# yjtang249/MIPSFusion

Hardware: NVIDIA B200
Metric: map_step_rays_per_s (higher is better)
Workload: dtype f32 (decoder contractions as bf16x3 hi/lo splits on tcgen05, fp32 accumulate; encodings, render, losses, Adam in fp32)

## Files before the change

mipsfusion_b200/csrc/field_kernels.cu:

```cuda
#include "field_bwd.cuh"
#include "field_launch.cuh"
#include "field_tc_launch.cuh"
#include "field_tc_bwd.cuh"
#include "field_tc_bwd2.cuh"
#include "field_tc_bwd3.cuh"

__device__ __forceinline__ void mlp_prepare_simt(const float* __restrict__ mlp, float* __restrict__ prep, int i) {
    if (i >= PREP_SIMT_SIZE) return;
    float v = 0.f;
    if (i < MF_MLP_PARAMS) {
        v = mlp[i];
    } else if (i >= PREP_F1) {
        int r;
        if (i < PREP_B1) {
            int off, K, Kreal;
            if (i < PREP_F2) { r = i - PREP_F1; off = OFF_W1; K = D_E; Kreal = D_E; }
            else if (i < PREP_F3) { r = i - PREP_F2; off = OFF_W2; K = D_H; Kreal = D_H; }
            else { r = i - PREP_F3; off = OFF_WS1; K = D_SDF_IN; Kreal = D_SDF_IN; }
            const int k = r >> 7, tx = (r >> 3) & 15, i8 = r & 7;
            const int n = tx + 16 * i8;
            v = (k < Kreal) ? mlp[off + n * K + k] : 0.f;
        } else {
            int off, K, KI;
            if (i < PREP_B2) { r = i - PREP_B1; off = OFF_W1; K = D_E; KI = 4; }
            else if (i < PREP_B3) { r = i - PREP_B2; off = OFF_W2; K = D_H; KI = 8; }
            else { r = i - PREP_B3; off = OFF_WS1; K = D_SDF_IN; KI = 6; }
            const int n = r / (16 * KI), rem = r % (16 * KI), tx = rem / KI, ii = rem % KI;
            const int k = tx + 16 * ii;
            v = (k < K) ? mlp[off + n * K + k] : 0.f;
        }
    }
    prep[i] = v;
}

__device__ __forceinline__ void mlp_prepare_tc(const float* __restrict__ mlp, uint8_t* __restrict__ img, int t) {
    if (t < 128 * 320) {
        const int n = t / 320, kk = t % 320;
        float w; int hi_off, lo_off, k;
        if (kk < 64) {
            k = kk; const int e = tc_e_slot_to_index(k);
            w = e >= 0 ? mlp[OFF_W1 + n * D_E + e] : 0.f;
            hi_off = IMG_W1_HI; lo_off = IMG_W1_LO;
        } else if (kk < 192) {
            k = kk - 64; w = mlp[OFF_W2 + n * D_H + k];
            hi_off = IMG_W2_HI; lo_off = IMG_W2_LO;
        } else {
            k = kk - 192; w = k < D_SDF_IN ? mlp[OFF_WS1 + n * D_SDF_IN + k] : 0.f;
            hi_off = IMG_W3_HI; lo_off = IMG_W3_LO;
        }
        const __nv_bfloat16 h = __float2bfloat16_rn(w);
        const __nv_bfloat16 l = __float2bfloat16_rn(w - __bfloat162float(h));
        const uint32_t off = (uint32_t)(k >> 6) * IMG_BLOCK + sw128_offset(n, k & 63);
        *reinterpret_cast<__nv_bfloat16*>(img + hi_off + off) = h;
        *reinterpret_cast<__nv_bfloat16*>(img + lo_off + off) = l;
    } else if (t < 128 * 320 + F_COUNT) {
        const int j = t - 128 * 320;
        float v = 0.f;
        if (j < F_B2) v = mlp[OFF_B1 + j];
        else if (j < F_BS1) v = mlp[OFF_B2 + (j - F_B2)];
        else if (j < F_WR_EMB) v = mlp[OFF_BS1 + (j - F_BS1)];
        else if (j < F_WR_E) { const int c = (j - F_WR_EMB) / 64, k = (j - F_WR_EMB) % 64; v = mlp[OFF_WR + c * D_RGB_IN + k]; }
        else if (j < F_BR) {
            const int c = (j - F_WR_E) / 64, e = tc_e_slot_to_index((j - F_WR_E) % 64);
            v = e >= 0 ? mlp[OFF_WR + c * D_RGB_IN + 64 + e] : 0.f;
        }
        else if (j < F_WS2) v = (j - F_BR) < 3 ? mlp[OFF_BR + (j - F_BR)] : 0.f;
        else if (j < F_BS2) v = mlp[OFF_WS2 + (j - F_WS2)];
        else v = (j - F_BS2) < 5 ? mlp[OFF_BS2 + (j - F_BS2)] : 0.f;
        reinterpret_cast<float*>(img + IMG_F32)[j] = v;
    }
}

constexpr int PREP_BLOCKS_SIMT = (PREP_SIMT_SIZE + 255) / 256;
constexpr int PREP_BLOCKS_TC = (128 * 320 + F_COUNT + 255) / 256;
__global__ void __launch_bounds__(256) mlp_prepare_kernel(const float* __restrict__ mlp, float* __restrict__ prep) {
    if (blockIdx.x < PREP_BLOCKS_SIMT) mlp_prepare_simt(mlp, prep, blockIdx.x * 256 + threadIdx.x);
    else mlp_prepare_tc(mlp, reinterpret_cast<uint8_t*>(prep + PREP_TC), (blockIdx.x - PREP_BLOCKS_SIMT) * 256 + threadIdx.x);
}

__global__ void __launch_bounds__(NT, 2) mlp_fwd_kernel(const float* embed, const float* embed_pos, const float* pts,
                                                        const float* __restrict__ prep, float* __restrict__ out, int64_t N) {
    extern __shared__ __align__(16) float sm[];
    const int64_t n_tiles = (N + TP - 1) / TP;
    for (int64_t tile = blockIdx.x; tile < n_tiles; tile += gridDim.x) {
        load_features_tile(embed, embed_pos, pts, tile, N, sm);
        __syncthreads();
        mlp_forward_tile<false>(prep, sm, sm + ROW_H1 * LDA);
        __syncthreads();
        store_raw_tile(sm + ROW_OUT * LDA, LDA, TP, out, tile, N, threadIdx.x, NT);
        __syncthreads();
    }
}

template <class Src, bool WANT_DX>
__global__ void __launch_bounds__(NT, 1) field_bwd_kernel(FieldDev f, Src src, const float* __restrict__ d_raw,
                                                          float* __restrict__ grad_grid, float* __restrict__ part,
                                                          float* __restrict__ d_pts, int64_t N_all, ActiveMap am) {
    extern __shared__ __align__(16) float sm[];
    float* gpart = part + (size_t)blockIdx.x * MF_MLP_PARAMS;
    for (int i = threadIdx.x; i < MF_MLP_PARAMS; i += NT) gpart[i] = 0.f;
    __syncthreads();
    const int64_t N = am.n(N_all);
    const int64_t n_tiles = (N + TP - 1) / TP;
    for (int64_t tile = blockIdx.x; tile < n_tiles; tile += gridDim.x) {
        encode_tile(f, src, tile, N, sm, am);
        __syncthreads();
        mlp_forward_tile<false>(f.prep, sm, sm + ROW_H3 * LDA);
        __syncthreads();
        head_backward_tile(d_raw, tile, N, sm, am);
        __syncthreads();
        mlp_backward_tile<WANT_DX>(f.prep, sm, gpart);
        encode_backward_tile<Src, WANT_DX>(f, src, tile, N, sm, grad_grid, d_pts, am);
        __syncthreads();
    }
}

template <class Src>
__global__ void __launch_bounds__(NT, 1) field_bwd_dx_kernel(FieldDev f, Src src, const float* __restrict__ d_raw,
                                                             float* __restrict__ d_pts, int64_t N_all, ActiveMap am) {
    extern __shared__ __align__(16) float sm[];
    const int64_t N = am.n(N_all);
    const int64_t n_tiles = (N + TP - 1) / TP;
    for (int64_t tile = blockIdx.x; tile < n_tiles; tile += gridDim.x) {
        encode_tile(f, src, tile, N, sm, am);
        __syncthreads();
        mlp_forward_tile<false>(f.prep, sm, sm + ROW_H3 * LDA);
        __syncthreads();
        head_backward_tile(d_raw, tile, N, sm, am);
        __syncthreads();
        mlp_backward_tile<true, false>(f.prep, sm, nullptr);
        encode_backward_tile<Src, true, false>(f, src, tile, N, sm, nullptr, d_pts, am);
        __syncthreads();
    }
}

template <bool WANT_DX>
__global__ void __launch_bounds__(NT, 1) mlp_bwd_kernel(const float* embed, const float* embed_pos, const float* pts,
                                                        const float* __restrict__ prep, const float* __restrict__ d_out,
                                                        float* __restrict__ part, float* __restrict__ d_embed,
                                                        float* __restrict__ d_embed_pos, float* __restrict__ d_pts, int64_t N) {
    extern __shared__ __align__(16) float sm[];
    float* gpart = part + (size_t)blockIdx.x * MF_MLP_PARAMS;
    for (int i = threadIdx.x; i < MF_MLP_PARAMS; i += NT) gpart[i] = 0.f;
    __syncthreads();
    const int64_t n_tiles = (N + TP - 1) / TP;
    for (int64_t tile = blockIdx.x; tile < n_tiles; tile += gridDim.x) {
        load_features_tile(embed, embed_pos, pts, tile, N, sm);
        __syncthreads();
        mlp_forward_tile<false>(prep, sm, sm + ROW_H3 * LDA);
        __syncthreads();
        head_backward_tile(d_out, tile, N, sm);
        __syncthreads();
        mlp_backward_tile<WANT_DX>(prep, sm, gpart);
        const float* E = sm + ROW_E * LDA; const float* G = sm + ROW_G * LDA;
        const int64_t base = tile * TP;
        const int nv = (int)min((int64_t)TP, N - base);
        if (d_embed)
            for (int idx = threadIdx.x; idx < nv * D_GRID; idx += NT)
                d_embed[base * D_GRID + idx] = G[(idx % D_GRID) * LDA + idx / D_GRID];
        if (WANT_DX) {
            if (d_embed_pos)
                for (int idx = threadIdx.x; idx < nv * D_FREQ; idx += NT)
                    d_embed_pos[base * D_FREQ + idx] = E[(3 + idx % D_FREQ) * LDA + idx / D_FREQ];
            if (d_pts)
                for (int idx = threadIdx.x; idx < nv * 3; idx += NT) d_pts[base * 3 + idx] = E[(idx % 3) * LDA + idx / 3];
        }
        __syncthreads();
    }
}

__global__ void __launch_bounds__(256) reduce_partials_kernel(const float* __restrict__ part, int n_cta, float* __restrict__ grad_mlp,
                                                              int transposed, const float* __restrict__ mlp) {
    __shared__ float acc[8][32];
    if (transposed == 2 && blockIdx.x == gridDim.x - 1) {
        __shared__ float dbs1[D_H], dbr[4];
        const int t = threadIdx.x;
        if (t < D_H + 3) {
            const int sidx = t < D_H ? OFF_BS1 + t : OFF_BR + (t - D_H);
            float s = 0.f;
            for (int c = 0; c < n_cta; ++c) s += __ldg(&part[(size_t)c * MF_MLP_PARAMS + sidx]);
            if (t < D_H) dbs1[t] = s; else dbr[t - D_H] = s;
        }
        __syncthreads();
        if (t < D_H) {
            float s = 0.f;
            if (t < D_SDF_EMB) {
                for (int m = 0; m < D_H; ++m) s = fmaf(dbs1[m], __ldg(&mlp[OFF_WS1 + m * D_SDF_IN + t]), s);
            } else {
                for (int c = 0; c < 3; ++c) s = fmaf(dbr[c], __ldg(&mlp[OFF_WR + c * D_RGB_IN + (t - D_SDF_EMB)]), s);
            }
            grad_mlp[OFF_B2 + t] += s;
        }
        return;
    }
    const int lane = threadIdx.x & 31, j = threadIdx.x >> 5;
    const int sidx = blockIdx.x * 32 + lane;
    const bool on = sidx < MF_MLP_PARAMS;
    float s = 0.f;
    if (on) {
#pragma unroll 4
        for (int c = j; c < n_cta; c += 8) s += __ldg(&part[(size_t)c * MF_MLP_PARAMS + sidx]);
    }
    acc[j][lane] = s;
    __syncthreads();
    const bool b2_entry = transposed == 2 && sidx >= OFF_B2 && sidx < OFF_B2 + D_H;
    if (j == 0 && on && !b2_entry) {
        const float tot = ((acc[0][lane] + acc[1][lane]) + (acc[2][lane] + acc[3][lane])) + ((acc[4][lane] + acc[5][lane]) + (acc[6][lane] + acc[7][lane]));
        int dst = sidx;
        if (transposed) {
            if (sidx < OFF_B1) { const int r = sidx - OFF_W1; dst = OFF_W1 + (r % D_H) * D_E + r / D_H; }
            else if (sidx >= OFF_W2 && sidx < OFF_B2) { const int r = sidx - OFF_W2; dst = OFF_W2 + (r % D_H) * D_H + r / D_H; }
            else if (sidx >= OFF_WS1 && sidx < OFF_BS1) { const int r = sidx - OFF_WS1; dst = OFF_WS1 + (r % D_H) * D_SDF_IN + r / D_H; }
        }
        grad_mlp[dst] += tot;
    }
}

__global__ void ray_grad_reduce_kernel(const float* __restrict__ d_pts, const float* __restrict__ z,
                                       float* __restrict__ d_o, float* __restrict__ d_d, int64_t R, int S) {
    const int64_t r = (int64_t)blockIdx.x * (blockDim.x >> 5) + (threadIdx.x >> 5);
    const int lane = threadIdx.x & 31;
    if (r >= R) return;
    float so[3] = {0.f, 0.f, 0.f}, sd[3] = {0.f, 0.f, 0.f};
    for (int s = lane; s < S; s += 32) {
        const float zz = z[r * S + s];
#pragma unroll
        for (int k = 0; k < 3; ++k) {
            const float g = d_pts[(r * S + s) * 3 + k];
            so[k] += g; sd[k] = fmaf(zz, g, sd[k]);
        }
    }
#pragma unroll
    for (int k = 0; k < 3; ++k) { so[k] = warp_sum(so[k]); sd[k] = warp_sum(sd[k]); }
    if (lane == 0) {
#pragma unroll
        for (int k = 0; k < 3; ++k) { d_o[r * 3 + k] = so[k]; d_d[r * 3 + k] = sd[k]; }
    }
}

__global__ void hashgrid_fwd_kernel(FieldDev f, const float* __restrict__ x, float* __restrict__ out,
                                    uint32_t* __restrict__ idx_dump, int64_t N) {
    const int64_t t = (int64_t)blockIdx.x * blockDim.x + threadIdx.x;
    const int L = f.n_levels;
    if (t >= N * L) return;
    const int64_t i = t / L; const int l = (int)(t % L);
    const float xv[3] = {x[i * 3], x[i * 3 + 1], x[i * 3 + 2]};
    uint32_t idx[8];
    const float2 v = grid_level_fwd(xv, reinterpret_cast<const float2*>(f.grid), level_info(f, l), idx);
    reinterpret_cast<float2*>(out)[t] = v;
    if (idx_dump) {
#pragma unroll
        for (int c = 0; c < 8; ++c) idx_dump[t * 8 + c] = idx[c];
    }
}

template <bool WANT_DX>
__global__ void hashgrid_bwd_kernel(FieldDev f, const float* __restrict__ x, const float* __restrict__ dy,
                                    float* __restrict__ grad, float* __restrict__ dx_out, int64_t N) {
    const int64_t t = (int64_t)blockIdx.x * blockDim.x + threadIdx.x;
    const int L = f.n_levels;
    const bool active = t < N * L;
    const int64_t i = active ? t / L : 0; const int l = (int)(t % L);
    float dx[3] = {0.f, 0.f, 0.f};
    if (active) {
        const float xv[3] = {x[i * 3], x[i * 3 + 1], x[i * 3 + 2]};
        const float2 g = reinterpret_cast<const float2*>(dy)[t];
        grid_level_bwd<WANT_DX>(xv, g, reinterpret_cast<const float2*>(f.grid), grad, level_info(f, l), dx);
    }
    if (WANT_DX) {
#pragma unroll
        for (int d = 0; d < 3; ++d)
#pragma unroll
            for (int o = 8; o > 0; o >>= 1) dx[d] += __shfl_xor_sync(0xffffffffu, dx[d], o);
        if (active && l == 0) { dx_out[i * 3] = dx[0]; dx_out[i * 3 + 1] = dx[1]; dx_out[i * 3 + 2] = dx[2]; }
    }
}

__global__ void freq_fwd_kernel(const float* __restrict__ x, float* __restrict__ out, int D, int K, int64_t N) {
    const int64_t t = (int64_t)blockIdx.x * blockDim.x + threadIdx.x;
    const int W = D * K * 2;
    if (t >= N * W) return;
    const int64_t i = t / W; const int j = (int)(t % W);
    const int d = j / (2 * K), k = (j / 2) % K, s = j & 1;
    out[t] = sinf(freq_arg(x[i * D + d], k, s));
}

__global__ void freq_bwd_kernel(const float* __restrict__ x, const float* __restrict__ dy, float* __restrict__ dx,
                                int D, int K, int64_t N) {
    const int64_t t = (int64_t)blockIdx.x * blockDim.x + threadIdx.x;
    if (t >= N * D) return;
    const int64_t i = t / D; const int d = (int)(t % D);
    const float xv = x[t];
    float s = 0.f;
    for (int k = 0; k < K; ++k)
        for (int ph = 0; ph < 2; ++ph)
            s += dy[i * (D * K * 2) + d * 2 * K + 2 * k + ph] * cosf(freq_arg(xv, k, ph)) * ldexpf(3.14159274101257324f, k);
    dx[t] = s;
}

int mf_field_to_dev(const mf_field* f, FieldDev* d) {
    if (!f || !f->grid || !f->mlp_prep) { mf_set_error("mf_field: null grid/mlp_prep"); return MF_ERR_INVALID; }
    if (f->meta.n_levels != 16 || f->meta.n_features != 2) {
        mf_set_error("fused field kernels are built for 16 levels x 2 features (got %d x %d)", f->meta.n_levels, f->meta.n_features);
        return MF_ERR_UNSUPPORTED;
    }
    d->grid = f->grid; d->prep = f->mlp_prep; d->feat = nullptr;
    d->tc_img = reinterpret_cast<const uint8_t*>(f->mlp_prep + PREP_TC);
    for (int k = 0; k < 3; ++k) { d->na[k] = f->norm_a[k]; d->nb[k] = f->norm_b[k]; }
    d->nf = f->norm_factor;
    for (int l = 0; l < f->meta.n_levels; ++l)
        if (f->meta.offset[l] & 1u) { mf_set_error("mf_field: level offsets must be even (16-byte reductions)"); return MF_ERR_INVALID; }
    d->impl = f->decoder_impl == 0 ? mf_decoder_impl() : (f->decoder_impl == 1 ? 1 : 0);
    d->n_levels = f->meta.n_levels;
    for (int l = 0; l < MF_MAX_LEVELS; ++l) {
        d->scale[l] = f->meta.scale[l]; d->res[l] = f->meta.resolution[l]; d->size[l] = f->meta.size[l];
        d->offset[l] = f->meta.offset[l]; d->hashed[l] = f->meta.hashed[l];
    }
    return MF_OK;
}

static int meta_to_dev(const mf_grid_meta* m, const float* grid, FieldDev* d) {
    if (!m || m->n_levels < 1 || m->n_levels > MF_MAX_LEVELS || m->n_features != 2) {
        mf_set_error("hash grid: need 1..16 levels and 2 features per level");
        return MF_ERR_UNSUPPORTED;
    }
    memset(d, 0, sizeof(*d));
    d->grid = grid; d->n_levels = m->n_levels; d->nf = 1.0;
    for (int l = 0; l < m->n_levels; ++l) {
        d->scale[l] = m->scale[l]; d->res[l] = m->resolution[l]; d->size[l] = m->size[l];
        d->offset[l] = m->offset[l]; d->hashed[l] = m->hashed[l];
    }
    return MF_OK;
}

MF_API int mf_hashgrid_meta(int log2_T, int n_levels, int n_features, int base_res, double per_level_scale, mf_grid_meta* m) {
    MF_CHECK_ARG(m != nullptr);
    MF_CHECK_ARG(n_levels >= 1 && n_levels <= MF_MAX_LEVELS);
    MF_CHECK_ARG(log2_T >= 1 && log2_T <= 30);
    memset(m, 0, sizeof(*m));
    m->n_levels = n_levels; m->n_features = n_features; m->log2_hashmap_size = log2_T; m->base_resolution = base_res;
    const float log2_pls = log2f((float)per_level_scale);
    uint32_t off = 0;
    for (int l = 0; l < n_levels; ++l) {
        const float arg = (float)l * log2_pls;
        const float s = (float)exp2((double)arg) * (float)base_res - 1.0f;
        const uint32_t r = (uint32_t)ceilf(s) + 1u;
        const uint32_t max_params = UINT32_MAX / 2;
        uint32_t n = (powf((float)r, 3.0f) > (float)max_params) ? max_params : r * r * r;
        n = (n + 7u) / 8u * 8u;
        const uint32_t cap = 1u << log2_T;
        if (n > cap) n = cap;
        uint32_t stride = 1;
        for (int d = 0; d < 3 && stride <= n; ++d) stride *= r;
        m->scale[l] = s; m->resolution[l] = r; m->size[l] = n; m->offset[l] = off; m->hashed[l] = (n < stride) ? 1u : 0u;
        off += n;
    }
    m->offset[n_levels] = off;
    return MF_OK;
}

MF_API int mf_hashgrid_fwd(const float* x, const float* grid, const mf_grid_meta* meta, float* out, uint32_t* idx_dump,
                           int64_t N, void* stream) {
    MF_CHECK_ARG(N >= 0);
    if (N == 0) return MF_OK;
    MF_CHECK_ARG(x && grid && out);
    FieldDev d; int rc = meta_to_dev(meta, grid, &d); if (rc) return rc;
    const int64_t T = N * d.n_levels;
    hashgrid_fwd_kernel<<<(unsigned)((T + 255) / 256), 256, 0, (cudaStream_t)stream>>>(d, x, out, idx_dump, N);
    MF_LAUNCH_CHECK();
    return MF_OK;
}

MF_API int mf_hashgrid_bwd(const float* x, const float* dL_dy, const float* grid, const mf_grid_meta* meta,
                           float* grad_grid, float* dL_dx, int64_t N, void* stream) {
    MF_CHECK_ARG(N >= 0);
    if (N == 0) return MF_OK;
    MF_CHECK_ARG(x && dL_dy && grid && grad_grid);
    MF_CHECK_ARG(((uintptr_t)grad_grid & 15) == 0);
    FieldDev d; int rc = meta_to_dev(meta, grid, &d); if (rc) return rc;
    for (int l = 0; l < d.n_levels; ++l) MF_CHECK_ARG((d.offset[l] & 1u) == 0);
    if (dL_dx && d.n_levels != 16) { mf_set_error("mf_hashgrid_bwd: input gradient needs 16 levels"); return MF_ERR_UNSUPPORTED; }
    const int64_t T = N * d.n_levels;
    const unsigned blocks = (unsigned)((T + 255) / 256);
    if (dL_dx) hashgrid_bwd_kernel<true><<<blocks, 256, 0, (cudaStream_t)stream>>>(d, x, dL_dy, grad_grid, dL_dx, N);
    else hashgrid_bwd_kernel<false><<<blocks, 256, 0, (cudaStream_t)stream>>>(d, x, dL_dy, grad_grid, nullptr, N);
    MF_LAUNCH_CHECK();
    return MF_OK;
}

MF_API int mf_freq_fwd(const float* x, float* out, int n_dims, int n_frequencies, int64_t N, void* stream) {
    MF_CHECK_ARG(N >= 0 && n_dims > 0 && n_frequencies > 0);
    if (N == 0) return MF_OK;
    MF_CHECK_ARG(x && out);
    const int64_t T = N * n_dims * n_frequencies * 2;
    freq_fwd_kernel<<<(unsigned)((T + 255) / 256), 256, 0, (cudaStream_t)stream>>>(x, out, n_dims, n_frequencies, N);
    MF_LAUNCH_CHECK();
    return MF_OK;
}

MF_API int mf_freq_bwd(const float* x, const float* dL_dy, float* dL_dx, int n_dims, int n_frequencies, int64_t N, void* stream) {
    MF_CHECK_ARG(N >= 0 && n_dims > 0 && n_frequencies > 0);
    if (N == 0) return MF_OK;
    MF_CHECK_ARG(x && dL_dy && dL_dx);
    const int64_t T = N * n_dims;
    freq_bwd_kernel<<<(unsigned)((T + 255) / 256), 256, 0, (cudaStream_t)stream>>>(x, dL_dy, dL_dx, n_dims, n_frequencies, N);
    MF_LAUNCH_CHECK();
    return MF_OK;
}

MF_API int64_t mf_mlp_prep_size(void) { return PREP_SIZE; }

MF_API int mf_mlp_prepare(const float* mlp, float* mlp_prep, void* stream) {
    MF_CHECK_ARG(mlp && mlp_prep);
    mlp_prepare_kernel<<<PREP_BLOCKS_SIMT + PREP_BLOCKS_TC, 256, 0, (cudaStream_t)stream>>>(mlp, mlp_prep);
    MF_LAUNCH_CHECK();
    return MF_OK;
}

MF_API int64_t mf_mlp_grad_workspace_size(void) { return (int64_t)mf_sm_count_cached() * MF_MLP_PARAMS; }

MF_API int mf_mlp_fwd(const float* embed, const float* embed_pos, const float* pts, const float* mlp_prep, float* out,
                      int64_t N, void* stream) {
    MF_CHECK_ARG(N >= 0);
    if (N == 0) return MF_OK;
    MF_CHECK_ARG(embed && embed_pos && pts && mlp_prep && out);
    int rc = set_smem(mlp_fwd_kernel, SMEM_FWD); if (rc) return rc;
    mlp_fwd_kernel<<<persistent_grid(N, 2), NT, SMEM_FWD, (cudaStream_t)stream>>>(embed, embed_pos, pts, mlp_prep, out, N);
    MF_LAUNCH_CHECK();
    return MF_OK;
}

MF_API int mf_mlp_bwd(const float* embed, const float* embed_pos, const float* pts, const float* mlp_prep,
                      const float* d_out, float* grad_mlp, float* d_embed, float* d_embed_pos, float* d_pts,
                      float* workspace, int64_t N, void* stream) {
    MF_CHECK_ARG(N >= 0);
    if (N == 0) return MF_OK;
    MF_CHECK_ARG(embed && embed_pos && pts && mlp_prep && d_out && grad_mlp && workspace);
    const bool want_dx = d_embed_pos || d_pts;
    const int grid = persistent_grid(N, 1);
    cudaStream_t st = (cudaStream_t)stream;
    if (want_dx) {
        int rc = set_smem(mlp_bwd_kernel<true>, SMEM_BWD); if (rc) return rc;
        mlp_bwd_kernel<true><<<grid, NT, SMEM_BWD, st>>>(embed, embed_pos, pts, mlp_prep, d_out, workspace, d_embed, d_embed_pos, d_pts, N);
    } else {
        int rc = set_smem(mlp_bwd_kernel<false>, SMEM_BWD); if (rc) return rc;
        mlp_bwd_kernel<false><<<grid, NT, SMEM_BWD, st>>>(embed, embed_pos, pts, mlp_prep, d_out, workspace, d_embed, nullptr, nullptr, N);
    }
    MF_LAUNCH_CHECK();
    reduce_partials_kernel<<<(MF_MLP_PARAMS + 31) / 32, 256, 0, st>>>(workspace, grid, grad_mlp, 0, nullptr);
    MF_LAUNCH_CHECK();
    return MF_OK;
}

constexpr int ACT_BLK = 1024;

__global__ void __launch_bounds__(ACT_BLK) active_count_kernel(const float* __restrict__ d_raw, int64_t N,
                                                               uint32_t* __restrict__ flags, int* __restrict__ blk_cnt) {
    const int64_t i = (int64_t)blockIdx.x * ACT_BLK + threadIdx.x;
    bool on = false;
    if (i < N) {
        const float2* g = reinterpret_cast<const float2*>(d_raw + i * MF_RAW_DIM);
#pragma unroll
        for (int k = 0; k < MF_RAW_DIM / 2; ++k) { const float2 v = __ldg(g + k); on |= (v.x != 0.f) | (v.y != 0.f); }
    }
    const uint32_t word = __ballot_sync(0xffffffffu, on);
    if ((threadIdx.x & 31) == 0) flags[i >> 5] = word;
    const int total = __syncthreads_count(on);
    if (threadIdx.x == 0) blk_cnt[blockIdx.x] = total;
}

__global__ void __launch_bounds__(ACT_BLK) active_fill_kernel(const uint32_t* __restrict__ flags, const int* __restrict__ blk_cnt,
                                                              int* __restrict__ idx, int* __restrict__ n_active) {
    __shared__ int wsum[32];
    __shared__ int base_s;
    const int tid = threadIdx.x, lane = tid & 31, warp = tid >> 5;
    int part = 0;
    for (int j = tid; j < (int)blockIdx.x; j += ACT_BLK) part += blk_cnt[j];
#pragma unroll
    for (int o = 16; o > 0; o >>= 1) part += __shfl_xor_sync(0xffffffffu, part, o);
    if (lane == 0) wsum[warp] = part;
    __syncthreads();
    if (warp == 0) {
        int v = wsum[lane];
#pragma unroll
        for (int o = 16; o > 0; o >>= 1) v += __shfl_xor_sync(0xffffffffu, v, o);
        if (lane == 0) base_s = v;
    }
    __syncthreads();
    const int base = base_s;
    const int64_t i = (int64_t)blockIdx.x * ACT_BLK + tid;
    const uint32_t word = flags[i >> 5];
    __syncthreads();
    if (lane == 0) wsum[warp] = __popc(word);
    __syncthreads();
    if (warp == 0) {
        const int c = wsum[lane];
        int v = c;
#pragma unroll
        for (int o = 1; o < 32; o <<= 1) { const int t = __shfl_up_sync(0xffffffffu, v, o); if (lane >= o) v += t; }
        wsum[lane] = v - c;
        if (lane == 31 && blockIdx.x == gridDim.x - 1) *n_active = base + v;
    }
    __syncthreads();
    if ((word >> lane) & 1u) idx[base + wsum[warp] + __popc(word & ((1u << lane) - 1u))] = (int)i;
}

static inline int64_t act_blocks(int64_t N) { return (N + ACT_BLK - 1) / ACT_BLK; }
static inline int64_t act_scratch_words(int64_t N) { return N + act_blocks(N) * 33 + 4; }

static int compact_active_points(const float* d_raw, int64_t N, float* scratch, ActiveMap* am, cudaStream_t st) {
    if ((uintptr_t)d_raw & 7) { mf_set_error("backward: the upstream gradient must be 8-byte aligned"); return MF_ERR_INVALID; }
    if (N >= (int64_t)1 << 31) { mf_set_error("backward: more than 2^31 points"); return MF_ERR_INVALID; }
    const int64_t nb = act_blocks(N);
    int* idx = reinterpret_cast<int*>(scratch);
    uint32_t* flags = reinterpret_cast<uint32_t*>(idx + N);
    int* blk_cnt = reinterpret_cast<int*>(flags + nb * 32);
    int* count = blk_cnt + nb;
    active_count_kernel<<<(unsigned)nb, ACT_BLK, 0, st>>>(d_raw, N, flags, blk_cnt);
    MF_LAUNCH_CHECK();
    active_fill_kernel<<<(unsigned)nb, ACT_BLK, 0, st>>>(flags, blk_cnt, idx, count);
    MF_LAUNCH_CHECK();
    am->idx = idx; am->count = count;
    return MF_OK;
}

static inline int64_t cta_scratch_words() { return (int64_t)mf_sm_count_cached() * b2::SCR_CTA_WORDS; }

MF_API int64_t mf_field_bwd_workspace_size(int64_t n_points, int want_point_grads) {
    if (n_points < 0) n_points = 0;
    return mf_mlp_grad_workspace_size() + (want_point_grads ? 3 * n_points : 0) + act_scratch_words(n_points) + cta_scratch_words();
}

template <class Src>
static int launch_field_bwd(const FieldDev& d, const Src& src, const float* d_raw, float* grad_grid, float* grad_mlp,
                            float* d_pts, float* workspace, float* scratch, int64_t N, cudaStream_t st) {
    ActiveMap am{nullptr, nullptr};
    int rc0 = compact_active_points(d_raw, N, scratch, &am, st); if (rc0) return rc0;
    if (d_pts) MF_CUDA(cudaMemsetAsync(d_pts, 0, (size_t)N * 3 * sizeof(float), st));
    const bool params = grad_grid != nullptr;
    if (!params && !d_pts) {
        mf_set_error("backward without parameter gradients needs a ray / point gradient output");
        return MF_ERR_INVALID;
    }
    if (!params && d.impl == 1) {
        const int grid = persistent_grid(N, 1);
        int rc = set_smem(field_bwd_dx_kernel<Src>, SMEM_BWD); if (rc) return rc;
        field_bwd_dx_kernel<Src><<<grid, NT, SMEM_BWD, st>>>(d, src, d_raw, d_pts, N, am);
        MF_LAUNCH_CHECK();
        return MF_OK;
    }
    if (d.impl != 1) {
        const int64_t tiles = (N + TC_TP - 1) / TC_TP;
        const int64_t cap = mf_sm_count_cached();
        const int grid = (int)(tiles < cap ? (tiles > 0 ? tiles : 1) : cap);
        mf_ktimer_begin(1, st);
        if (!params) {
            int rc = set_smem(field_bwd_tc_kernel<Src, true, false>, SMEM_TC_BWD); if (rc) return rc;
            field_bwd_tc_kernel<Src, true, false><<<grid, TC_NT, SMEM_TC_BWD, st>>>(d, src, d_raw, nullptr, nullptr, d_pts, N, am, mf_tc_error_flag(), mf_tc_profile_buffer());
            mf_ktimer_end(1, st);
            MF_LAUNCH_CHECK();
            return MF_OK;
        }
        if (!d_pts && mf_bwd_impl() != 1) {
            uint32_t* cta_scr = reinterpret_cast<uint32_t*>(scratch + act_scratch_words(N));
            if (mf_bwd_impl() == 3 && d.feat) {
                int rc = set_smem(field_bwd_tc3_kernel<Src>, b3::SMEM); if (rc) return rc;
                field_bwd_tc3_kernel<Src><<<grid, b3::B3_NT, b3::SMEM, st>>>(d, src, d_raw, grad_grid, workspace, cta_scr, N, am, mf_tc_error_flag(), mf_tc_profile_buffer());
            } else {
                int rc = set_smem(field_bwd_tc2_kernel<Src>, b2::SMEM); if (rc) return rc;
                field_bwd_tc2_kernel<Src><<<grid, b2::B2_NT, b2::SMEM, st>>>(d, src, d_raw, grad_grid, workspace, cta_scr, N, am, mf_tc_error_flag(), mf_tc_profile_buffer(),
                                                                             mf_bwd_impl() == 2 ? 0 : 1);
            }
            mf_ktimer_end(1, st);
            MF_LAUNCH_CHECK();
            reduce_partials_kernel<<<(MF_MLP_PARAMS + 31) / 32 + 1, 256, 0, st>>>(workspace, grid, grad_mlp, 2, d.prep);
            MF_LAUNCH_CHECK();
            return MF_OK;
        }
        if (d_pts) {
            int rc = set_smem(field_bwd_tc_kernel<Src, true>, SMEM_TC_BWD); if (rc) return rc;
            field_bwd_tc_kernel<Src, true><<<grid, TC_NT, SMEM_TC_BWD, st>>>(d, src, d_raw, grad_grid, workspace, d_pts, N, am, mf_tc_error_flag(), mf_tc_profile_buffer());
        } else {
            int rc = set_smem(field_bwd_tc_kernel<Src, false>, SMEM_TC_BWD); if (rc) return rc;
            field_bwd_tc_kernel<Src, false><<<grid, TC_NT, SMEM_TC_BWD, st>>>(d, src, d_raw, grad_grid, workspace, nullptr, N, am, mf_tc_error_flag(), mf_tc_profile_buffer());
        }
        mf_ktimer_end(1, st);
        MF_LAUNCH_CHECK();
        reduce_partials_kernel<<<(MF_MLP_PARAMS + 31) / 32, 256, 0, st>>>(workspace, grid, grad_mlp, 1, nullptr);
        MF_LAUNCH_CHECK();
        return MF_OK;
    }
    const int grid = persistent_grid(N, 1);
    if (d_pts) {
        int rc = set_smem(field_bwd_kernel<Src, true>, SMEM_BWD); if (rc) return rc;
        field_bwd_kernel<Src, true><<<grid, NT, SMEM_BWD, st>>>(d, src, d_raw, grad_grid, workspace, d_pts, N, am);
    } else {
        int rc = set_smem(field_bwd_kernel<Src, false>, SMEM_BWD); if (rc) return rc;
        field_bwd_kernel<Src, false><<<grid, NT, SMEM_BWD, st>>>(d, src, d_raw, grad_grid, workspace, nullptr, N, am);
    }
    MF_LAUNCH_CHECK();
    reduce_partials_kernel<<<(MF_MLP_PARAMS + 31) / 32, 256, 0, st>>>(workspace, grid, grad_mlp, 0, nullptr);
    MF_LAUNCH_CHECK();
    return MF_OK;
}

MF_API int mf_field_query(const float* pts, const mf_field* field, int normalize, float* out, int64_t N, void* stream) {
    MF_CHECK_ARG(N >= 0);
    if (N == 0) return MF_OK;
    MF_CHECK_ARG(pts && out);
    FieldDev d; int rc = mf_field_to_dev(field, &d); if (rc) return rc;
    SrcPoints src{pts, normalize};
    return launch_field_fwd_auto<SrcPoints, EpiRaw, false>(d, src, EpiRaw{out}, N, (cudaStream_t)stream);
}

MF_API int mf_field_query_bwd(const float* pts, const mf_field* field, int normalize, const float* d_out, float* grad_grid,
                              float* grad_mlp, float* d_pts, float* workspace, int64_t N, void* stream) {
    MF_CHECK_ARG(N >= 0);
    if (N == 0) return MF_OK;
    MF_CHECK_ARG(pts && d_out && workspace);
    MF_CHECK_ARG((grad_grid == nullptr) == (grad_mlp == nullptr));
    MF_CHECK_ARG(grad_grid || d_pts);
    MF_CHECK_ARG(((uintptr_t)grad_grid & 15) == 0);
    FieldDev d; int rc = mf_field_to_dev(field, &d); if (rc) return rc;
    SrcPoints src{pts, normalize};
    return launch_field_bwd(d, src, d_out, grad_grid, grad_mlp, d_pts, workspace, workspace + mf_mlp_grad_workspace_size(), N,
                            (cudaStream_t)stream);
}

MF_API int64_t mf_feat_cache_size(int64_t n_points) {
    return ((n_points + TC_TP - 1) / TC_TP) * (int64_t)FEAT_TILE_WORDS * 4;
}

MF_API int mf_field_query_rays(const float* rays_o, const float* rays_d, const float* z, const mf_field* field, float* raw,
                               void* feat, int64_t R, int S, void* stream) {
    MF_CHECK_ARG(R >= 0 && S > 0);
    if (R == 0) return MF_OK;
    MF_CHECK_ARG(rays_o && rays_d && z && raw);
    FieldDev d; int rc = mf_field_to_dev(field, &d); if (rc) return rc;
    d.feat = (uint32_t*)feat;
    SrcRays src{rays_o, rays_d, z, S};
    return launch_field_fwd_auto<SrcRays, EpiRaw, false>(d, src, EpiRaw{raw}, R * S, (cudaStream_t)stream, nullptr, false, 0);
}

MF_API int mf_field_query_rays_bwd(const float* rays_o, const float* rays_d, const float* z, const mf_field* field,
                                   const float* d_raw, const void* feat, float* grad_grid, float* grad_mlp, float* d_rays_o,
                                   float* d_rays_d, float* workspace, int64_t R, int S, void* stream) {
    MF_CHECK_ARG(R >= 0 && S > 0);
    if (R == 0) return MF_OK;
    MF_CHECK_ARG(rays_o && rays_d && z && d_raw && workspace);
    MF_CHECK_ARG((grad_grid == nullptr) == (grad_mlp == nullptr));
    MF_CHECK_ARG(((uintptr_t)grad_grid & 15) == 0);
    MF_CHECK_ARG((d_rays_o == nullptr) == (d_rays_d == nullptr));
    FieldDev d; int rc = mf_field_to_dev(field, &d); if (rc) return rc;
    d.feat = (uint32_t*)feat;
    SrcRays src{rays_o, rays_d, z, S};
    cudaStream_t st = (cudaStream_t)stream;
    float* d_pts = d_rays_o ? workspace + mf_mlp_grad_workspace_size() : nullptr;
    float* scratch = workspace + mf_mlp_grad_workspace_size() + (d_rays_o ? 3 * R * S : 0);
    rc = launch_field_bwd(d, src, d_raw, grad_grid, grad_mlp, d_pts, workspace, scratch, R * S, st);
    if (rc) return rc;
    if (d_rays_o) {
        ray_grad_reduce_kernel<<<(unsigned)((R + 7) / 8), 256, 0, st>>>(d_pts, z, d_rays_o, d_rays_d, R, S);
        MF_LAUNCH_CHECK();
    }
    return MF_OK;
}
```

mipsfusion_b200/csrc/field_tc.cuh:

```cuda
#pragma once
#include "grid_encode.cuh"
#include "umma.cuh"

constexpr int TC_TP = 128;
constexpr int TC_NT = 512;
constexpr int TC_LD = TC_TP + 4;
constexpr int FEAT_WORDS = 24;
constexpr int FEAT_TILE_WORDS = 4 * FEAT_WORDS * TC_TP;

constexpr int IMG_BLOCK = 16384;
constexpr int IMG_W1_HI = 0;
constexpr int IMG_W1_LO = IMG_W1_HI + IMG_BLOCK;
constexpr int IMG_W2_HI = IMG_W1_LO + IMG_BLOCK;
constexpr int IMG_W2_LO = IMG_W2_HI + 2 * IMG_BLOCK;
constexpr int IMG_W3_HI = IMG_W2_LO + 2 * IMG_BLOCK;
constexpr int IMG_W3_LO = IMG_W3_HI + 2 * IMG_BLOCK;
constexpr int IMG_F32 = IMG_W3_LO + 2 * IMG_BLOCK;
constexpr int F_B1 = 0, F_B2 = 128, F_BS1 = 256;
constexpr int F_WR_EMB = 384;
constexpr int F_WR_E = F_WR_EMB + 192;
constexpr int F_BR = F_WR_E + 192;
constexpr int F_WS2 = F_BR + 4;
constexpr int F_BS2 = F_WS2 + 640;
constexpr int F_COUNT = F_BS2 + 8;
constexpr int IMG_BYTES = IMG_F32 + F_COUNT * 4;
static_assert(IMG_BYTES % 16 == 0, "image is copied with 16-byte loads");

__host__ __device__ inline int tc_e_slot_to_index(int slot) {
    const int q = slot >> 4, jj = slot & 15;
    if (jj < 12) return 3 + 12 * q + jj;
    if (q == 0 && jj < 15) return jj - 12;
    return -1;
}

__host__ __device__ inline uint32_t sw128_offset(int row, int k) {
    return (uint32_t)((row >> 3) * 1024 + (row & 7) * 128 + ((((k >> 3) ^ (row & 7)) & 7) << 4) + (k & 7) * 2);
}

constexpr int TM_D = 0;
constexpr int TM_A_HI = 128;
constexpr int TM_A_LO = 192;
constexpr int TM_G_HI = 256;
constexpr int TM_G_LO = 272;
constexpr int TM_COLS = 512;

constexpr int TCS_IMG = 0;
constexpr int TCS_PART = ((IMG_BYTES + 127) / 128) * 128;
constexpr int TCS_OUT = TCS_PART + 40 * TC_LD * 4;
constexpr int TCS_BAR = TCS_OUT + 10 * TC_LD * 4;
constexpr int TCS_BYTES = TCS_BAR + 32;
constexpr size_t SMEM_TC = TCS_BYTES + 1024;

struct TcCtx {
    uint8_t* img; float* part; float* out; uint64_t* bar; uint32_t* tmem_ptr;
    uint32_t tmem_base, lane_base, phase;
    const float* fw;
};

__device__ __forceinline__ void tc_setup(TcCtx& c, uint8_t* smem_raw, const uint8_t* __restrict__ img_g) {
    uint8_t* base = (uint8_t*)(((uintptr_t)smem_raw + 1023) & ~(uintptr_t)1023);
    c.img = base + TCS_IMG; c.part = (float*)(base + TCS_PART); c.out = (float*)(base + TCS_OUT);
    c.bar = (uint64_t*)(base + TCS_BAR); c.tmem_ptr = (uint32_t*)(base + TCS_BAR + 8);
    c.fw = (const float*)(c.img + IMG_F32);
    const int tid = threadIdx.x;
    for (int i = tid; i < IMG_BYTES / 16; i += blockDim.x)
        reinterpret_cast<uint4*>(c.img)[i] = __ldg(reinterpret_cast<const uint4*>(img_g) + i);
    umma::fence_proxy_async();
    if ((tid >> 5) == 0) umma::tmem_alloc<TM_COLS>(c.tmem_ptr);
    if (tid == 0) { umma::mbar_init(c.bar, 1); umma::fence_barrier_init(); }
    umma::fence_before_sync();
    __syncthreads();
    umma::fence_after_sync();
    c.tmem_base = *c.tmem_ptr;
    c.lane_base = c.tmem_base + ((uint32_t)(((tid >> 5) & 3) * 32) << 16);
    c.phase = 0;
}

__device__ __forceinline__ void tc_teardown(TcCtx& c) {
    umma::fence_before_sync();
    __syncthreads();
    if ((threadIdx.x >> 5) == 0) umma::tmem_dealloc<TM_COLS>(c.tmem_base);
}

template <class ColFn>
__device__ __forceinline__ void tc_layer_mma(const TcCtx& c, int img_hi, int img_lo, int KS, ColFn a_col) {
    constexpr uint32_t idesc = umma::idesc_bf16(128, 128, 0, 0);
    const uint32_t d = c.tmem_base + TM_D;
    const uint32_t w_hi = umma::smem_u32(c.img + img_hi), w_lo = umma::smem_u32(c.img + img_lo);
    uint32_t acc = 0;
#pragma unroll 1
    for (int pass = 0; pass < 3; ++pass) {
        const bool a_is_lo = pass == 2, w_is_lo = pass == 1;
#pragma unroll 1
        for (int ks = 0; ks < KS; ++ks) {
            const uint32_t a = c.tmem_base + (uint32_t)a_col(ks, a_is_lo);
            const uint32_t wb = (w_is_lo ? w_lo : w_hi) + (uint32_t)((ks >> 2) * IMG_BLOCK + (ks & 3) * 32);
            umma::mma_ts(d, a, umma::smem_desc_sw128(wb, 16, 1024), idesc, acc);
            acc = 1;
        }
    }
}

template <class ColFn>
__device__ __forceinline__ bool tc_run_layer(TcCtx& c, int img_hi, int img_lo, int KS, ColFn a_col) {
    umma::wait_st();
    umma::fence_before_sync();
    __syncthreads();
    if (threadIdx.x == 0) {
        umma::fence_after_sync();
        tc_layer_mma(c, img_hi, img_lo, KS, a_col);
        umma::commit(c.bar);
    }
    const bool ok = umma::mbar_wait(c.bar, c.phase);
    c.phase ^= 1;
    umma::fence_after_sync();
    return ok;
}

__device__ __forceinline__ void tc_load_acc(const TcCtx& c, int q, float (&v)[32]) {
    uint32_t r[32];
    umma::tmem_ld32(c.lane_base + TM_D + 32 * q, r);
    umma::wait_ld();
#pragma unroll
    for (int i = 0; i < 32; ++i) v[i] = __uint_as_float(r[i]);
}

__device__ __forceinline__ void tc_store_act32(const TcCtx& c, int q, const float (&v)[32]) {
    uint32_t hi[16], lo[16];
#pragma unroll
    for (int i = 0; i < 16; ++i) umma::split2(v[2 * i], v[2 * i + 1], hi[i], lo[i]);
    umma::tmem_st16(c.lane_base + TM_A_HI + 16 * q, hi);
    umma::tmem_st16(c.lane_base + TM_A_LO + 16 * q, lo);
}

template <class Src, bool SDF_ONLY>
__device__ __forceinline__ void tc_encode_tile(const TcCtx& c, const FieldDev& f, const Src& src, int64_t tile, int64_t N) {
    const int tid = threadIdx.x, p = tid & (TC_TP - 1), q = tid >> 7;
    const int64_t i = tile * TC_TP + p;
    const bool valid = i < N;
    float x[3] = {0.f, 0.f, 0.f};
    if (valid) src.point(i, f, x);
    float e[16];
#pragma unroll
    for (int jj = 0; jj < 12; ++jj) {
        const int j = q * 12 + jj, d = j >> 4, k = (j & 15) >> 1, s = j & 1;
        e[jj] = sin_reduced(freq_arg(x[d], k, s));
    }
    e[12] = q == 0 ? x[0] : 0.f; e[13] = q == 0 ? x[1] : 0.f; e[14] = q == 0 ? x[2] : 0.f; e[15] = 0.f;
    {
        uint32_t hi[8], lo[8];
#pragma unroll
        for (int t = 0; t < 8; ++t) umma::split2(e[2 * t], e[2 * t + 1], hi[t], lo[t]);
        umma::tmem_st8(c.lane_base + TM_A_HI + 8 * q, hi);
        umma::tmem_st8(c.lane_base + TM_A_LO + 8 * q, lo);
        if (f.feat) {
            uint32_t* fo = f.feat + (size_t)tile * FEAT_TILE_WORDS + (size_t)q * FEAT_WORDS * TC_TP + p;
#pragma unroll
            for (int t = 0; t < 8; ++t) { fo[t * TC_TP] = hi[t]; fo[(8 + t) * TC_TP] = lo[t]; }
        }
    }
    if (!SDF_ONLY) {
        const float* wre = c.fw + F_WR_E + 16 * q;
        float r[3] = {0.f, 0.f, 0.f};
#pragma unroll
        for (int t = 0; t < 16; ++t)
#pragma unroll
            for (int ch = 0; ch < 3; ++ch) r[ch] = fmaf(wre[ch * 64 + t], e[t], r[ch]);
#pragma unroll
        for (int ch = 0; ch < 3; ++ch) c.part[(q * 3 + ch) * TC_LD + p] = r[ch];
    }
    const float2* grid2 = reinterpret_cast<const float2*>(f.grid);
    float g[8];
#pragma unroll
    for (int ll = 0; ll < 4; ++ll) {
        float2 v = make_float2(0.f, 0.f);
        if (valid) v = grid_level_fwd(x, grid2, level_info(f, q * 4 + ll), nullptr);
        g[2 * ll] = v.x; g[2 * ll + 1] = v.y;
    }
    {
        uint32_t hi[4], lo[4];
#pragma unroll
        for (int t = 0; t < 4; ++t) umma::split2(g[2 * t], g[2 * t + 1], hi[t], lo[t]);
        umma::tmem_st4(c.lane_base + TM_G_HI + 4 * q, hi);
        umma::tmem_st4(c.lane_base + TM_G_LO + 4 * q, lo);
        if (f.feat) {
            uint32_t* fo = f.feat + (size_t)tile * FEAT_TILE_WORDS + (size_t)q * FEAT_WORDS * TC_TP + p;
#pragma unroll
            for (int t = 0; t < 4; ++t) { fo[(16 + t) * TC_TP] = hi[t]; fo[(20 + t) * TC_TP] = lo[t]; }
        }
    }
}

template <bool SDF_ONLY>
__device__ __forceinline__ bool tc_mlp_forward_tile(TcCtx& c) {
    const int tid = threadIdx.x, p = tid & (TC_TP - 1), q = tid >> 7;
    bool ok = true;
    float v[32];
    ok &= tc_run_layer(c, IMG_W1_HI, IMG_W1_LO, 4, [](int ks, bool lo) { return (lo ? TM_A_LO : TM_A_HI) + 8 * ks; });
    tc_load_acc(c, q, v);
#pragma unroll
    for (int i = 0; i < 32; ++i) v[i] = fmaxf(v[i] + c.fw[F_B1 + 32 * q + i], 0.f);
    tc_store_act32(c, q, v);
    ok &= tc_run_layer(c, IMG_W2_HI, IMG_W2_LO, 8, [](int ks, bool lo) { return (lo ? TM_A_LO : TM_A_HI) + 8 * ks; });
    tc_load_acc(c, q, v);
#pragma unroll
    for (int i = 0; i < 32; ++i) v[i] += c.fw[F_B2 + 32 * q + i];
    if (q < 2) {
        tc_store_act32(c, q, v);
    } else if (!SDF_ONLY) {
        const float* wr = c.fw + F_WR_EMB + 32 * (q - 2);
        float r[3] = {0.f, 0.f, 0.f};
#pragma unroll
        for (int i = 0; i < 32; ++i)
#pragma unroll
            for (int ch = 0; ch < 3; ++ch) r[ch] = fmaf(wr[ch * 64 + i], v[i], r[ch]);
#pragma unroll
        for (int ch = 0; ch < 3; ++ch) c.part[(12 + (q - 2) * 3 + ch) * TC_LD + p] = r[ch];
    }
    ok &= tc_run_layer(c, IMG_W3_HI, IMG_W3_LO, 6, [](int ks, bool lo) {
        return ks < 4 ? (lo ? TM_A_LO : TM_A_HI) + 8 * ks : (lo ? TM_G_LO : TM_G_HI) + 8 * (ks - 4);
    });
    tc_load_acc(c, q, v);
    {
        float s[N_CLASS] = {0.f, 0.f, 0.f, 0.f, 0.f};
        const float* ws2 = c.fw + F_WS2 + 32 * q;
#pragma unroll
        for (int i = 0; i < 32; ++i) {
            const float h = fmaxf(v[i] + c.fw[F_BS1 + 32 * q + i], 0.f);
#pragma unroll
            for (int ch = 0; ch < N_CLASS; ++ch) s[ch] = fmaf(ws2[ch * 128 + i], h, s[ch]);
        }
#pragma unroll
        for (int ch = 0; ch < N_CLASS; ++ch) c.part[(18 + q * 5 + ch) * TC_LD + p] = s[ch];
    }
    umma::fence_before_sync();
    __syncthreads();
    if (q == 0) {
        const float* P = c.part;
        float zl[N_CLASS], rgb[3];
#pragma unroll
        for (int ch = 0; ch < N_CLASS; ++ch)
            zl[ch] = c.fw[F_BS2 + ch] + ((P[(18 + ch) * TC_LD + p] + P[(23 + ch) * TC_LD + p]) + (P[(28 + ch) * TC_LD + p] + P[(33 + ch) * TC_LD + p]));
#pragma unroll
        for (int ch = 0; ch < 3; ++ch)
            rgb[ch] = SDF_ONLY ? 0.f
                               : c.fw[F_BR + ch] + (((P[ch * TC_LD + p] + P[(3 + ch) * TC_LD + p]) + (P[(6 + ch) * TC_LD + p] + P[(9 + ch) * TC_LD + p])) +
                                                    (P[(12 + ch) * TC_LD + p] + P[(15 + ch) * TC_LD + p]));
        float mx = zl[0];
#pragma unroll
        for (int ch = 1; ch < N_CLASS; ++ch) mx = fmaxf(mx, zl[ch]);
        float pr[N_CLASS], se = 0.f;
#pragma unroll
        for (int ch = 0; ch < N_CLASS; ++ch) { pr[ch] = expf(zl[ch] - mx); se += pr[ch]; }
        float ent = 0.f, ex = 0.f;
#pragma unroll
        for (int ch = 0; ch < N_CLASS; ++ch) {
            pr[ch] = pr[ch] / se;
            ent += pr[ch] * log2f(pr[ch] + 1e-5f);
            ex += pr[ch] * (float)ch;
        }
        float* O = c.out;
        O[0 * TC_LD + p] = rgb[0]; O[1 * TC_LD + p] = rgb[1]; O[2 * TC_LD + p] = rgb[2];
        O[3 * TC_LD + p] = (ex / 4.0f - 0.5f) * 2.0f;
        O[4 * TC_LD + p] = -1.0f * ent;
#pragma unroll
        for (int ch = 0; ch < N_CLASS; ++ch) O[(5 + ch) * TC_LD + p] = pr[ch];
    }
    return ok;
}

template <class Src, class Epi, bool SDF_ONLY>
__global__ void __launch_bounds__(TC_NT, 1) field_fwd_tc_kernel(FieldDev f, Src src, Epi epi, int64_t N,
                                                                const unsigned int* __restrict__ n_dev,
                                                                const uint8_t* __restrict__ img, int* __restrict__ err,
                                                                long long* __restrict__ prof) {
    extern __shared__ uint8_t smem_raw[];
#define TC_MARK(k) do { if (prof && threadIdx.x == 0 && blockIdx.x == 0 && tile == (int64_t)gridDim.x) prof[32 + (k)] = clock64(); } while (0)
    if (n_dev) N = (int64_t)*n_dev;
    TcCtx c;
    tc_setup(c, smem_raw, img);
    bool ok = true;
    const int64_t n_tiles = (N + TC_TP - 1) / TC_TP;
    for (int64_t tile = blockIdx.x; tile < n_tiles; tile += gridDim.x) {
        TC_MARK(0);
        tc_encode_tile<Src, SDF_ONLY>(c, f, src, tile, N);
        TC_MARK(1);
        ok &= tc_mlp_forward_tile<SDF_ONLY>(c);
        TC_MARK(2);
        __syncthreads();
        epi.store(c.out, TC_LD, TC_TP, tile, N, threadIdx.x, TC_NT);
        __syncthreads();
        TC_MARK(3);
    }
    if (!ok && err) atomicExch(err, 1);
    tc_teardown(c);
}
```

mipsfusion_b200/csrc/field_tc3.cuh:

```cuda
#pragma once
#include "field_tc.cuh"

constexpr int T3_GT = 256;
constexpr int T3_D = 0, T3_A_HI = 128, T3_A_LO = 192, T3_STG = 256, T3_STG_COLS = 96;
constexpr int T3_E_HI = 0, T3_E_LO = 32, T3_G_HI = 64, T3_G_LO = 80;
constexpr int T3_CPART_ROWS = 6;
constexpr int T3_PART_ROWS = 13;
constexpr int T3S_CPART = ((IMG_BYTES + 127) / 128) * 128;
constexpr int T3S_PART = T3S_CPART + 2 * T3_CPART_ROWS * TC_LD * 4;
constexpr int T3S_OUT = T3S_PART + T3_PART_ROWS * TC_LD * 4;
constexpr int T3S_BAR = T3S_OUT + MF_RAW_DIM * TC_LD * 4;
constexpr size_t SMEM_TC3 = T3S_BAR + 64 + 1024;
static_assert(SMEM_TC3 <= 227 * 1024, "shared memory budget");

__device__ __forceinline__ void t3_cons_sync() { asm volatile("bar.sync 1, %0;" ::"n"(T3_GT) : "memory"); }

struct T3Cons {
    uint8_t* img; const float* fw; float* part; float* out; uint64_t* bar;
    uint32_t tmem, lane_base, phase;
    int tid;
    bool ok;
};

template <int KS, int N_OUT = 128, class ColFn, class AfterFn>
__device__ __forceinline__ void t3_run_layer(T3Cons& c, int img_hi, int img_lo, ColFn a_col, AfterFn after_issue) {
    umma::wait_st();
    umma::fence_before_sync();
    t3_cons_sync();
    if (c.tid == 0) {
        umma::fence_after_sync();
        constexpr uint32_t idesc = umma::idesc_bf16(128, N_OUT, 0, 0);
        const uint64_t dh = umma::smem_desc_sw128(umma::smem_u32(c.img + img_hi), 16, 1024);
        const uint64_t dl = umma::smem_desc_sw128(umma::smem_u32(c.img + img_lo), 16, 1024);
#pragma unroll
        for (int pass = 0; pass < 3; ++pass) {
#pragma unroll
            for (int ks = 0; ks < KS; ++ks) {
                const uint32_t off = (uint32_t)(((ks >> 2) * IMG_BLOCK + (ks & 3) * 32) >> 4);
                umma::mma_ts(c.tmem + T3_D, c.tmem + (uint32_t)a_col(ks, pass == 2), (pass == 1 ? dl : dh) + off, idesc, (pass | ks) ? 1u : 0u);
            }
        }
        umma::commit(c.bar);
        after_issue();
    }
    c.ok &= umma::mbar_wait(c.bar, c.phase);
    c.phase ^= 1;
    umma::fence_after_sync();
}

__device__ __forceinline__ void t3_load32(const T3Cons& c, int col, float (&v)[32]) {
    uint32_t r[32];
    umma::tmem_ld32(c.lane_base + (uint32_t)col, r);
    umma::wait_ld();
#pragma unroll
    for (int i = 0; i < 32; ++i) v[i] = __uint_as_float(r[i]);
}
__device__ __forceinline__ void t3_store32(const T3Cons& c, int f0, const float (&v)[32]) {
    uint32_t hi[16], lo[16];
#pragma unroll
    for (int i = 0; i < 16; ++i) umma::split2(v[2 * i], v[2 * i + 1], hi[i], lo[i]);
    umma::tmem_st16(c.lane_base + (uint32_t)(T3_A_HI + f0 / 2), hi);
    umma::tmem_st16(c.lane_base + (uint32_t)(T3_A_LO + f0 / 2), lo);
}

template <class Src, class Epi, bool SDF_ONLY>
__global__ void __launch_bounds__(2 * T3_GT, 1) field_fwd_tc3_kernel(FieldDev f, Src src, Epi epi, int64_t N,
                                                                     const unsigned int* __restrict__ n_dev,
                                                                     const uint8_t* __restrict__ img, int* __restrict__ err,
                                                                     long long* __restrict__ prof, int* __restrict__ tile_ctr = nullptr) {
    extern __shared__ uint8_t smem_raw[];
    __shared__ uint32_t tmem_ptr_s;
#define T3_MARK(slot) do { if (prof && blockIdx.x == 0 && tid == 0 && k == 2) prof[slot] = clock64(); } while (0)
    if (n_dev) N = (int64_t)*n_dev;
    if (prof && blockIdx.x == 0 && threadIdx.x == 0) prof[29] = clock64();
    if (prof && threadIdx.x == 0 && blockIdx.x < 256) prof[64 + 2 * blockIdx.x] = mf_globaltimer();
    uint8_t* base = (uint8_t*)(((uintptr_t)smem_raw + 1023) & ~(uintptr_t)1023);
    uint64_t* bars = (uint64_t*)(base + T3S_BAR);
    if ((threadIdx.x >> 5) == 0) umma::tmem_alloc<512>(&tmem_ptr_s);
    if (threadIdx.x == 0) {
        umma::mbar_init(bars + 0, 1);
        umma::mbar_init(bars + 1, T3_GT); umma::mbar_init(bars + 2, T3_GT);
        umma::mbar_init(bars + 3, 1); umma::mbar_init(bars + 4, 1);
        umma::mbar_init(bars + 7, 1);
        umma::fence_barrier_init();
        constexpr uint32_t CHUNK = 32768;
        asm volatile("mbarrier.arrive.expect_tx.shared::cta.b64 _, [%0], %1;" ::"r"(umma::smem_u32(bars + 7)), "r"((uint32_t)IMG_BYTES) : "memory");
        for (uint32_t off = 0; off < (uint32_t)IMG_BYTES; off += CHUNK) {
            const uint32_t nb = (uint32_t)IMG_BYTES - off < CHUNK ? (uint32_t)IMG_BYTES - off : CHUNK;
            asm volatile("cp.async.bulk.shared::cluster.global.mbarrier::complete_tx::bytes [%0], [%1], %2, [%3];"
                         ::"r"(umma::smem_u32(base + off)), "l"(img + off), "r"(nb), "r"(umma::smem_u32(bars + 7)) : "memory");
        }
    }
    umma::fence_before_sync();
    __syncthreads();
    umma::fence_after_sync();
    bool img_ok = umma::mbar_wait(bars + 7, 0);
    const uint32_t tmem = tmem_ptr_s;
    const bool producer = threadIdx.x < T3_GT;
    const int tid = threadIdx.x & (T3_GT - 1), p = tid & 127, h = tid >> 7;
    const uint32_t lane_base = tmem + ((uint32_t)(((tid >> 5) & 3) * 32) << 16);
    const float* fw = (const float*)(base + IMG_F32);
    const int64_t n_tiles = (N + TC_TP - 1) / TC_TP;
    bool ok = img_ok;
    volatile int* tq = reinterpret_cast<volatile int*>(base + T3S_BAR + 40);
    if (threadIdx.x < 4) tq[threadIdx.x] = 0;

    if (producer) {
        const float2* grid2 = reinterpret_cast<const float2*>(f.grid);
        for (uint32_t k = 0;; ++k) {
            const int s = (int)(k & 1u);
            const uint32_t stg = lane_base + (uint32_t)(T3_STG + T3_STG_COLS * s);
            float* cpart = (float*)(base + T3S_CPART) + s * T3_CPART_ROWS * TC_LD;
            T3_MARK(40);
            if (prof && blockIdx.x == 0 && tid == 0 && k < 12) prof[16 + k] = clock64();
            const int64_t tile_e = k < 2 ? (int64_t)blockIdx.x + (int64_t)k * gridDim.x : (int64_t)tq[k & 3u];
            float x[3] = {0.f, 0.f, 0.f};
            if (tile_e >= 0 && tile_e < n_tiles && tile_e * TC_TP + p < N) src.point(tile_e * TC_TP + p, f, x);
            ok &= umma::mbar_wait(bars + 3 + s, ((k >> 1) & 1u) ^ 1u);
            umma::fence_after_sync();
            const int64_t tile = k < 2 ? tile_e : (int64_t)tq[k & 3u];
            if (tile >= n_tiles) break;
            if (tid == 0) {
                const int64_t t2 = tile_ctr ? 2 * (int64_t)gridDim.x + atomicAdd(tile_ctr, 1) : tile + 2 * (int64_t)gridDim.x;
                tq[(k + 2u) & 3u] = (int)(t2 < n_tiles ? t2 : n_tiles);
            }
            const int64_t i = tile * TC_TP + p;
            const bool valid = i < N;
            if (tile != tile_e) {
                x[0] = x[1] = x[2] = 0.f;
                if (valid) src.point(i, f, x);
            }
            T3_MARK(41);
            float r[3] = {0.f, 0.f, 0.f};
#pragma unroll
            for (int sg = 0; sg < 2; ++sg) {
                const int qq = 2 * h + sg;
                float e[16];
#pragma unroll
                for (int jj = 0; jj < 12; ++jj) {
                    const int j = qq * 12 + jj, d = j >> 4, kk = (j & 15) >> 1, ph = j & 1;
                    e[jj] = sin_reduced(freq_arg(x[d], kk, ph));
                }
                e[12] = qq == 0 ? x[0] : 0.f; e[13] = qq == 0 ? x[1] : 0.f; e[14] = qq == 0 ? x[2] : 0.f; e[15] = 0.f;
                uint32_t hi[8], lo[8];
#pragma unroll
                for (int t = 0; t < 8; ++t) umma::split2(e[2 * t], e[2 * t + 1], hi[t], lo[t]);
                umma::tmem_st8(stg + T3_E_HI + 8 * qq, hi);
                umma::tmem_st8(stg + T3_E_LO + 8 * qq, lo);
                if (f.feat) {
                    uint32_t* fo = f.feat + (size_t)tile * FEAT_TILE_WORDS + (size_t)qq * FEAT_WORDS * TC_TP + p;
#pragma unroll
                    for (int t = 0; t < 8; ++t) { fo[t * TC_TP] = hi[t]; fo[(8 + t) * TC_TP] = lo[t]; }
                }
                if (!SDF_ONLY) {
                    const float* wre = fw + F_WR_E + 16 * qq;
#pragma unroll
                    for (int t = 0; t < 16; ++t)
#pragma unroll
                        for (int ch = 0; ch < 3; ++ch) r[ch] = fmaf(wre[ch * 64 + t], e[t], r[ch]);
                }
            }
            if (!SDF_ONLY) {
#pragma unroll
                for (int ch = 0; ch < 3; ++ch) cpart[(h * 3 + ch) * TC_LD + p] = r[ch];
            }
            T3_MARK(42);
#pragma unroll 1
            for (int sg = 0; sg < 2; ++sg) {
                float gf[8];
#pragma unroll 2
                for (int ll = 0; ll < 4; ++ll) {
                    float2 v2 = make_float2(0.f, 0.f);
                    if (valid) v2 = grid_level_fwd(x, grid2, level_info(f, 8 * h + 4 * sg + ll), nullptr);
                    gf[2 * ll] = v2.x; gf[2 * ll + 1] = v2.y;
                }
                uint32_t ghi[4], glo[4];
#pragma unroll
                for (int t = 0; t < 4; ++t) umma::split2(gf[2 * t], gf[2 * t + 1], ghi[t], glo[t]);
                umma::tmem_st4(stg + T3_G_HI + 8 * h + 4 * sg, ghi);
                umma::tmem_st4(stg + T3_G_LO + 8 * h + 4 * sg, glo);
                if (f.feat) {
                    uint32_t* fo = f.feat + (size_t)tile * FEAT_TILE_WORDS + (size_t)(2 * h + sg) * FEAT_WORDS * TC_TP + p;
#pragma unroll
                    for (int t = 0; t < 4; ++t) { fo[(16 + t) * TC_TP] = ghi[t]; fo[(20 + t) * TC_TP] = glo[t]; }
                }
            }
            T3_MARK(43);
            umma::wait_st();
            umma::fence_before_sync();
            umma::mbar_arrive(bars + 1 + s);
            T3_MARK(44);
        }
    } else {
        T3Cons c;
        c.img = base; c.fw = fw; c.part = (float*)(base + T3S_PART); c.out = (float*)(base + T3S_OUT); c.bar = bars;
        c.tmem = tmem; c.lane_base = lane_base; c.phase = 0; c.tid = tid; c.ok = ok;
        float v[32];
        for (uint32_t k = 0;; ++k) {
            const int64_t tile = k < 2 ? (int64_t)blockIdx.x + (int64_t)k * gridDim.x : (int64_t)tq[k & 3u];
            if (tile >= n_tiles) break;
            const int s = (int)(k & 1u);
            const int stg = T3_STG + T3_STG_COLS * s;
            const float* cpart = (const float*)(base + T3S_CPART) + s * T3_CPART_ROWS * TC_LD;
            T3_MARK(48);
            c.ok &= umma::mbar_wait(bars + 1 + s, (k >> 1) & 1u);
            umma::fence_after_sync();
            T3_MARK(49);
            float rgb_e[3] = {0.f, 0.f, 0.f};
            if (!SDF_ONLY && h == 0) {
#pragma unroll
                for (int ch = 0; ch < 3; ++ch) rgb_e[ch] = cpart[ch * TC_LD + p] + cpart[(3 + ch) * TC_LD + p];
            }
            t3_run_layer<4>(c, IMG_W1_HI, IMG_W1_LO, [stg](int ks, bool lo) { return stg + (lo ? T3_E_LO : T3_E_HI) + 8 * ks; }, []() {});
            T3_MARK(50);
#pragma unroll 1
            for (int half = 0; half < 2; ++half) {
                const int f0 = 64 * h + 32 * half;
                t3_load32(c, T3_D + f0, v);
                const float4* b4 = reinterpret_cast<const float4*>(c.fw + F_B1 + f0);
#pragma unroll
                for (int k4 = 0; k4 < 8; ++k4) {
                    const float4 b = b4[k4];
                    v[4 * k4] = fmaxf(v[4 * k4] + b.x, 0.f); v[4 * k4 + 1] = fmaxf(v[4 * k4 + 1] + b.y, 0.f);
                    v[4 * k4 + 2] = fmaxf(v[4 * k4 + 2] + b.z, 0.f); v[4 * k4 + 3] = fmaxf(v[4 * k4 + 3] + b.w, 0.f);
                }
                t3_store32(c, f0, v);
            }
            T3_MARK(51);
            if (SDF_ONLY) {
                t3_run_layer<8, 64>(c, IMG_W2_HI, IMG_W2_LO, [](int ks, bool lo) { return (lo ? T3_A_LO : T3_A_HI) + 8 * ks; }, []() {});
                T3_MARK(52);
                const int f0 = 32 * h;
                t3_load32(c, T3_D + f0, v);
                const float4* b4 = reinterpret_cast<const float4*>(c.fw + F_B2 + f0);
#pragma unroll
                for (int k4 = 0; k4 < 8; ++k4) {
                    const float4 b = b4[k4];
                    v[4 * k4] += b.x; v[4 * k4 + 1] += b.y; v[4 * k4 + 2] += b.z; v[4 * k4 + 3] += b.w;
                }
                t3_store32(c, f0, v);
            } else {
            t3_run_layer<8>(c, IMG_W2_HI, IMG_W2_LO, [](int ks, bool lo) { return (lo ? T3_A_LO : T3_A_HI) + 8 * ks; }, []() {});
            T3_MARK(52);
            {
                float r[3] = {0.f, 0.f, 0.f};
#pragma unroll 1
                for (int half = 0; half < 2; ++half) {
                    const int f0 = 64 * h + 32 * half;
                    t3_load32(c, T3_D + f0, v);
                    const float4* b4 = reinterpret_cast<const float4*>(c.fw + F_B2 + f0);
#pragma unroll
                    for (int k4 = 0; k4 < 8; ++k4) {
                        const float4 b = b4[k4];
                        v[4 * k4] += b.x; v[4 * k4 + 1] += b.y; v[4 * k4 + 2] += b.z; v[4 * k4 + 3] += b.w;
                    }
                    if (h == 0) {
                        t3_store32(c, f0, v);
                    } else {
#pragma unroll
                        for (int ch = 0; ch < 3; ++ch) {
                            const float4* w4 = reinterpret_cast<const float4*>(c.fw + F_WR_EMB + ch * 64 + 32 * half);
#pragma unroll
                            for (int k4 = 0; k4 < 8; ++k4) {
                                const float4 w = w4[k4];
                                r[ch] = fmaf(w.x, v[4 * k4], r[ch]); r[ch] = fmaf(w.y, v[4 * k4 + 1], r[ch]);
                                r[ch] = fmaf(w.z, v[4 * k4 + 2], r[ch]); r[ch] = fmaf(w.w, v[4 * k4 + 3], r[ch]);
                            }
                        }
                    }
                }
                if (h == 1) {
#pragma unroll
                    for (int ch = 0; ch < 3; ++ch) c.part[ch * TC_LD + p] = r[ch];
                }
            }
            }
            T3_MARK(53);
            uint64_t* empty = bars + 3 + s;
            t3_run_layer<6>(c, IMG_W3_HI, IMG_W3_LO,
                         [stg](int ks, bool lo) { return ks < 4 ? (lo ? T3_A_LO : T3_A_HI) + 8 * ks : stg + (lo ? T3_G_LO : T3_G_HI) + 8 * (ks - 4); },
                         [empty]() { umma::commit(empty); });
            T3_MARK(54);
            {
                float sl[N_CLASS] = {0.f, 0.f, 0.f, 0.f, 0.f};
#pragma unroll 1
                for (int half = 0; half < 2; ++half) {
                    const int f0 = 64 * h + 32 * half;
                    t3_load32(c, T3_D + f0, v);
                    const float4* b4 = reinterpret_cast<const float4*>(c.fw + F_BS1 + f0);
#pragma unroll
                    for (int k4 = 0; k4 < 8; ++k4) {
                        const float4 b = b4[k4];
                        v[4 * k4] = fmaxf(v[4 * k4] + b.x, 0.f); v[4 * k4 + 1] = fmaxf(v[4 * k4 + 1] + b.y, 0.f);
                        v[4 * k4 + 2] = fmaxf(v[4 * k4 + 2] + b.z, 0.f); v[4 * k4 + 3] = fmaxf(v[4 * k4 + 3] + b.w, 0.f);
                    }
#pragma unroll
                    for (int ch = 0; ch < N_CLASS; ++ch) {
                        const float4* w4 = reinterpret_cast<const float4*>(c.fw + F_WS2 + ch * 128 + f0);
#pragma unroll
                        for (int k4 = 0; k4 < 8; ++k4) {
                            const float4 w = w4[k4];
                            sl[ch] = fmaf(w.x, v[4 * k4], sl[ch]); sl[ch] = fmaf(w.y, v[4 * k4 + 1], sl[ch]);
                            sl[ch] = fmaf(w.z, v[4 * k4 + 2], sl[ch]); sl[ch] = fmaf(w.w, v[4 * k4 + 3], sl[ch]);
                        }
                    }
                }
#pragma unroll
                for (int ch = 0; ch < N_CLASS; ++ch) c.part[(3 + h * 5 + ch) * TC_LD + p] = sl[ch];
            }
            T3_MARK(55);
            umma::fence_before_sync();
            t3_cons_sync();
            if (h == 0) {
                const float* P = c.part;
                float zl[N_CLASS], rgb[3];
#pragma unroll
                for (int ch = 0; ch < N_CLASS; ++ch) zl[ch] = c.fw[F_BS2 + ch] + (P[(3 + ch) * TC_LD + p] + P[(8 + ch) * TC_LD + p]);
#pragma unroll
                for (int ch = 0; ch < 3; ++ch) rgb[ch] = SDF_ONLY ? 0.f : c.fw[F_BR + ch] + (rgb_e[ch] + P[ch * TC_LD + p]);
                float mx = zl[0];
#pragma unroll
                for (int ch = 1; ch < N_CLASS; ++ch) mx = fmaxf(mx, zl[ch]);
                float pr[N_CLASS], se = 0.f;
#pragma unroll
                for (int ch = 0; ch < N_CLASS; ++ch) { pr[ch] = expf(zl[ch] - mx); se += pr[ch]; }
                float ent = 0.f, ex = 0.f;
#pragma unroll
                for (int ch = 0; ch < N_CLASS; ++ch) {
                    pr[ch] = pr[ch] / se;
                    ent += pr[ch] * log2f(pr[ch] + 1e-5f);
                    ex += pr[ch] * (float)ch;
                }
                float* O = c.out;
                O[0 * TC_LD + p] = rgb[0]; O[1 * TC_LD + p] = rgb[1]; O[2 * TC_LD + p] = rgb[2];
                O[3 * TC_LD + p] = (ex / 4.0f - 0.5f) * 2.0f;
                O[4 * TC_LD + p] = -1.0f * ent;
#pragma unroll
                for (int ch = 0; ch < N_CLASS; ++ch) O[(5 + ch) * TC_LD + p] = pr[ch];
            }
            t3_cons_sync();
            T3_MARK(56);
            epi.store(c.out, TC_LD, TC_TP, tile, N, c.tid, T3_GT);
            t3_cons_sync();
            T3_MARK(57);
        }
        ok = c.ok;
    }
    if (!ok && err) atomicExch(err, 1);
    umma::fence_before_sync();
    __syncthreads();
    if (prof && blockIdx.x == 0 && threadIdx.x == 0) prof[28] = clock64();
    if (prof && threadIdx.x == 0 && blockIdx.x < 256) prof[65 + 2 * blockIdx.x] = mf_globaltimer();
    if (tile_ctr && threadIdx.x == 0 && atomicAdd(tile_ctr + 1, 1) == (int)gridDim.x - 1) {
        tile_ctr[0] = 0; tile_ctr[1] = 0;
        __threadfence();
    }
    if ((threadIdx.x >> 5) == 0) umma::tmem_dealloc<512>(tmem);
}
```

mipsfusion_b200/csrc/field_tc_bwd2.cuh:

```cuda
#pragma once
#include "field_tc_bwd.cuh"

namespace b2 {

constexpr int B2_NT = 512, CHAIN_NT = 256, WG_NT = 128, SC_NT = 128;
constexpr int QROWS = 32;
constexpr uint32_t QBLK = QROWS * 128;
constexpr int S_W = 0;
constexpr int W2H = 0, W2L = IMG_W2_LO - IMG_W2_HI, W3H = IMG_W3_HI - IMG_W2_HI, W3L = IMG_W3_LO - IMG_W2_HI;
constexpr int S_ST = IMG_F32 - IMG_W2_HI;
constexpr int ST_A = 0, ST_B = 4 * (int)QBLK, ST_BYTES = 8 * (int)QBLK;
constexpr int W1H = S_ST + IMG_W1_HI, W1L = S_ST + IMG_W1_LO;
constexpr int S_F32 = S_ST + 2 * ST_BYTES;
constexpr int S_PART = S_F32 + ((F_COUNT * 4 + 127) / 128) * 128;
constexpr int PART_ROWS = 10;
constexpr int S_BAR = S_PART + PART_ROWS * TC_LD * 4;
constexpr int S_BYTES = S_BAR + 256;
constexpr size_t SMEM = S_BYTES + 1024;
static_assert(SMEM <= 227 * 1024, "shared memory budget");
constexpr int T_D = 0, T_R1_HI = 128, T_R1_LO = 192, T_R2_HI = 256, T_R2_LO = 320, T_DW = 384;
constexpr int T_G_HI = T_R2_HI + 32, T_G_LO = T_R2_LO + 32;
constexpr int SCR_H1 = 0, SCR_H3 = 128, SCR_RGB = 256, SCR_U = 320, SCR_WORDS = 328;
constexpr int64_t SCR_CTA_WORDS = (int64_t)SCR_WORDS * TC_TP;
constexpr int REGS_CHAIN = 160, REGS_WGRAD = 88, REGS_SCATTER = 104;
enum { B_MMA = 0, B_DG3, B_DCONS, B_DWFREE, B_DWRDY, B_W1, B_IMG, B_FREE0, B_ISS0 = B_FREE0 + 4, B_COUNT = B_ISS0 + 4 };
constexpr int N_X3 = 112;

__device__ __forceinline__ void chain_sync() { asm volatile("bar.sync 1, %0;" ::"n"(CHAIN_NT) : "memory"); }
__device__ __forceinline__ void wg_sync() { asm volatile("bar.sync 2, %0;" ::"n"(WG_NT) : "memory"); }

struct Ctx {
    uint8_t* base; const float* fw; float* part; uint64_t* bars;
    uint32_t tmem, lane_base;
    bool ok;
};

template <int KS, class ColFn>
__device__ __forceinline__ void issue_fwd(const Ctx& c, int w_hi_off, int w_lo_off, ColFn a_col) {
    constexpr uint32_t idesc = umma::idesc_bf16(128, 128, 0, 0);
    const uint64_t dh = umma::smem_desc_sw128(umma::smem_u32(c.base + S_W + w_hi_off), 16, 1024);
    const uint64_t dl = umma::smem_desc_sw128(umma::smem_u32(c.base + S_W + w_lo_off), 16, 1024);
#pragma unroll
    for (int pass = 0; pass < 3; ++pass)
#pragma unroll
        for (int ks = 0; ks < KS; ++ks) {
            const uint32_t off = (uint32_t)(((ks >> 2) * IMG_BLOCK + (ks & 3) * 32) >> 4);
            umma::mma_ts(c.tmem + T_D, c.tmem + (uint32_t)a_col(ks, pass == 2), (pass == 1 ? dl : dh) + off, idesc, (pass | ks) ? 1u : 0u);
        }
}
template <int N_OUT>
__device__ __forceinline__ void issue_dgrad(const Ctx& c, int a_hi, int a_lo, int w_hi_off, int w_lo_off) {
    constexpr uint32_t idesc = umma::idesc_bf16(128, N_OUT, 0, 1);
    const uint64_t dh = umma::smem_desc_sw128(umma::smem_u32(c.base + S_W + w_hi_off), IMG_BLOCK, 1024);
    const uint64_t dl = umma::smem_desc_sw128(umma::smem_u32(c.base + S_W + w_lo_off), IMG_BLOCK, 1024);
#pragma unroll
    for (int pass = 0; pass < 3; ++pass)
#pragma unroll
        for (int ks = 0; ks < 8; ++ks)
            umma::mma_ts(c.tmem + T_D, c.tmem + (uint32_t)((pass == 2 ? a_lo : a_hi) + 8 * ks), (pass == 1 ? dl : dh) + (uint32_t)((ks * 2048) >> 4),
                         idesc, (pass | ks) ? 1u : 0u);
}

__device__ __forceinline__ void ld32f(uint32_t taddr, float (&v)[32]) {
    uint32_t r[32];
    umma::tmem_ld32(taddr, r);
    umma::wait_ld();
#pragma unroll
    for (int i = 0; i < 32; ++i) v[i] = __uint_as_float(r[i]);
}

__device__ __forceinline__ void st_op(const Ctx& c, int hi_col, int lo_col, int f0, const uint32_t (&hi)[16], const uint32_t (&lo)[16]) {
    umma::tmem_st16(c.lane_base + (uint32_t)(hi_col + f0 / 2), hi);
    umma::tmem_st16(c.lane_base + (uint32_t)(lo_col + f0 / 2), lo);
}
__device__ __forceinline__ void split32(const float (&v)[32], uint32_t (&hi)[16], uint32_t (&lo)[16]) {
#pragma unroll
    for (int i = 0; i < 16; ++i) umma::split2(v[2 * i], v[2 * i + 1], hi[i], lo[i]);
}

template <int OFF>
__device__ __forceinline__ void sts128(uint32_t addr, uint32_t a, uint32_t b, uint32_t c_, uint32_t d) {
    asm volatile("st.shared.v4.b32 [%0+%1], {%2, %3, %4, %5};" ::"r"(addr), "n"(OFF), "r"(a), "r"(b), "r"(c_), "r"(d) : "memory");
}
template <int TILE_OFF, int CC>
__device__ __forceinline__ void put32(const uint32_t (&P)[8], const uint32_t (&pk)[16]) {
#pragma unroll
    for (int c_ = 0; c_ < 4; ++c_) sts128<TILE_OFF>(P[4 * CC + c_], pk[4 * c_], pk[4 * c_ + 1], pk[4 * c_ + 2], pk[4 * c_ + 3]);
}
template <int TILE_OFF, int SG>
__device__ __forceinline__ void put16(const uint32_t (&P)[8], const uint32_t (&pk)[8]) {
#pragma unroll
    for (int c_ = 0; c_ < 2; ++c_) sts128<TILE_OFF>(P[2 * SG + c_], pk[4 * c_], pk[4 * c_ + 1], pk[4 * c_ + 2], pk[4 * c_ + 3]);
}
template <int TILE_OFF>
__device__ __forceinline__ void put64(const uint32_t (&P)[8], const uint32_t (&wh)[2][16], const uint32_t (&wl)[2][16]) {
    put32<TILE_OFF, 0>(P, wh[0]); put32<TILE_OFF, 1>(P, wh[1]);
    put32<TILE_OFF + 2 * (int)QBLK, 0>(P, wl[0]); put32<TILE_OFF + 2 * (int)QBLK, 1>(P, wl[1]);
}

__device__ __forceinline__ void scr_store(uint32_t* scr_p, int region, int lo_off, int w0, const uint32_t (&hi)[16], const uint32_t (&lo)[16]) {
#pragma unroll
    for (int t = 0; t < 16; ++t) {
        __stcg(scr_p + (size_t)(region + w0 + t) * TC_TP, hi[t]);
        __stcg(scr_p + (size_t)(region + lo_off + w0 + t) * TC_TP, lo[t]);
    }
}
__device__ __forceinline__ void scr_load(const uint32_t* scr_p, int region, int lo_off, int w0, uint32_t (&hi)[16], uint32_t (&lo)[16]) {
#pragma unroll
    for (int t = 0; t < 16; ++t) {
        hi[t] = __ldcg(scr_p + (size_t)(region + w0 + t) * TC_TP);
        lo[t] = __ldcg(scr_p + (size_t)(region + lo_off + w0 + t) * TC_TP);
    }
}

}

template <class Src>
__global__ void __launch_bounds__(b2::B2_NT, 1) field_bwd_tc2_kernel(FieldDev f, Src src, const float* __restrict__ d_raw,
                                                                  float* __restrict__ grad_grid, float* __restrict__ part,
                                                                  uint32_t* __restrict__ scratch, int64_t N_all, ActiveMap am,
                                                                  int* __restrict__ err, long long* __restrict__ prof, int agg) {
    using namespace b2;
    extern __shared__ uint8_t smem_raw[];
    const int tid = threadIdx.x, warp = tid >> 5;
    if (prof && tid == 0 && blockIdx.x < 256) prof[576 + 2 * blockIdx.x] = mf_globaltimer();
    float* gpart = part + (size_t)blockIdx.x * MF_MLP_PARAMS;
    for (int i = tid; i < MF_MLP_PARAMS; i += B2_NT) gpart[i] = 0.f;

    Ctx c;
    c.base = (uint8_t*)(((uintptr_t)smem_raw + 1023) & ~(uintptr_t)1023);
    c.fw = (const float*)(c.base + S_F32); c.part = (float*)(c.base + S_PART); c.bars = (uint64_t*)(c.base + S_BAR);
    uint32_t* tmem_ptr = (uint32_t*)(c.base + S_BAR + 8 * B_COUNT);
    if (warp == 0) umma::tmem_alloc<512>(tmem_ptr);
    if (tid == 0) {
        umma::mbar_init(c.bars + B_MMA, 1); umma::mbar_init(c.bars + B_DG3, 1); umma::mbar_init(c.bars + B_DCONS, SC_NT);
        umma::mbar_init(c.bars + B_DWFREE, WG_NT); umma::mbar_init(c.bars + B_DWRDY, 4); umma::mbar_init(c.bars + B_W1, 1);
        umma::mbar_init(c.bars + B_IMG, 1);
        for (int q = 0; q < 4; ++q) { umma::mbar_init(c.bars + B_FREE0 + q, 1); umma::mbar_init(c.bars + B_ISS0 + q, 1); }
        umma::fence_barrier_init();
        constexpr uint32_t W_BYTES = IMG_F32 - IMG_W2_HI, F_BYTES = F_COUNT * 4, CHUNK = 32768;
        asm volatile("mbarrier.arrive.expect_tx.shared::cta.b64 _, [%0], %1;" ::"r"(umma::smem_u32(c.bars + B_IMG)), "r"(W_BYTES + F_BYTES) : "memory");
        for (uint32_t off = 0; off < W_BYTES; off += CHUNK)
            asm volatile("cp.async.bulk.shared::cluster.global.mbarrier::complete_tx::bytes [%0], [%1], %2, [%3];"
                         ::"r"(umma::smem_u32(c.base + S_W + off)), "l"(f.tc_img + IMG_W2_HI + off), "r"(W_BYTES - off < CHUNK ? W_BYTES - off : CHUNK),
                           "r"(umma::smem_u32(c.bars + B_IMG)) : "memory");
        asm volatile("cp.async.bulk.shared::cluster.global.mbarrier::complete_tx::bytes [%0], [%1], %2, [%3];"
                     ::"r"(umma::smem_u32(c.base + S_F32)), "l"(f.tc_img + IMG_F32), "r"(F_BYTES), "r"(umma::smem_u32(c.bars + B_IMG)) : "memory");
    }
    umma::fence_before_sync();
    __syncthreads();
    umma::fence_after_sync();
    c.tmem = *tmem_ptr;
    c.lane_base = c.tmem + ((uint32_t)((warp & 3) * 32) << 16);
    c.ok = umma::mbar_wait(c.bars + B_IMG, 0);

    const int64_t N = am.n(N_all);
    const int64_t n_tiles = (N + TC_TP - 1) / TC_TP;
    const int p = tid & (TC_TP - 1);
#define B2_MARK(slot) do { if (prof && blockIdx.x == 0 && k == 1 && (ctid & 127) == 0) prof[slot] = clock64(); } while (0)

    const int ctid = tid - SC_NT;
    if (ctid >= 0 && ctid < CHAIN_NT) {
        asm volatile("setmaxnreg.inc.sync.aligned.u32 %0;" ::"n"(REGS_CHAIN));
        const int h = ctid >> 7;
        uint32_t ph_mma = 0;
        uint32_t k = 0;
        auto round = [&](auto issue) {
            umma::wait_st();
            umma::fence_before_sync();
            chain_sync();
            if (ctid == 0) { umma::fence_after_sync(); issue(); umma::commit(c.bars + B_MMA); }
            c.ok &= umma::mbar_wait_spin(c.bars + B_MMA, ph_mma);
            ph_mma ^= 1;
            umma::fence_after_sync();
        };
        const int row = p & (QROWS - 1), quarter = p >> 5, lane = tid & 31;
        uint32_t PA[8], PH[8], PQ[4];
#pragma unroll
        for (int j = 0; j < 8; ++j) {
            PA[j] = umma::smem_u32(c.base) + (uint32_t)(S_ST + (quarter & 1) * ST_BYTES) + (uint32_t)((row >> 3) * 1024 + (row & 7) * 128) +
                    (uint32_t)(((j ^ row) & 7) << 4);
            PH[j] = PA[j] + (uint32_t)h * QBLK;
        }
#pragma unroll
        for (int c_ = 0; c_ < 4; ++c_) PQ[c_] = h ? PA[4 + c_] : PA[c_];
        const uint64_t dA0 = umma::desc_mn(c.base + S_ST + (quarter & 1) * ST_BYTES + ST_A, 0, QBLK);
        const uint64_t dB0 = umma::desc_mn(c.base + S_ST + (quarter & 1) * ST_BYTES + ST_B, 0, QBLK);
        constexpr uint32_t LO_STEP = (2 * QBLK) >> 4, KS_STEP = (16 * 128) >> 4;
        auto prod_begin = [&](uint32_t prod) {
            c.ok &= umma::mbar_wait_spin(c.bars + B_FREE0 + ((quarter + 2) & 3), quarter >= 2 ? (prod & 1u) : ((prod + 1u) & 1u));
        };
        auto prod_end = [&](int PK, uint32_t prod, uint32_t lay) {
            umma::fence_proxy_async();
            asm volatile("bar.sync %0, 64;" ::"r"(3 + quarter) : "memory");
            if (h == 0 && lane == 0) {
                umma::fence_after_sync();
                if (quarter == 0) {
                    if (PK == 0 || PK == 2 || PK == 3) c.ok &= umma::mbar_wait_spin(c.bars + B_DWFREE, (lay + 1u) & 1u);
                } else {
                    c.ok &= umma::mbar_wait_spin(c.bars + B_ISS0 + quarter - 1, prod & 1u);
                }
                const int n_out = PK == 0 ? N_X3 : (PK == 2 ? D_H : (PK == 3 ? 64 : 16));
                const uint32_t idesc = umma::idesc_bf16(128, n_out, 1, 1);
                const uint32_t dcol = c.tmem + (uint32_t)(T_DW + (PK == 1 ? N_X3 : (PK == 4 ? 64 : 0)));
#pragma unroll
                for (int j = 0; j < 6; ++j) {
                    const int pass = j >> 1, ks = j & 1;
                    umma::mma_ss(dcol, dA0 + (uint64_t)((pass == 1 ? LO_STEP : 0) + ks * KS_STEP),
                                 dB0 + (uint64_t)((pass == 2 ? LO_STEP : 0) + ks * KS_STEP), idesc, (j == 0 && quarter == 0) ? 0u : 1u);
                }
                umma::mbar_arrive(c.bars + B_ISS0 + quarter);
                umma::commit(c.bars + B_FREE0 + quarter);
                if (PK == 1 || PK == 2 || PK == 4) umma::commit(c.bars + B_DWRDY);
            }
        };
        auto put_u = [&](const uint32_t (&uh)[4], const uint32_t (&ul)[4]) {
            if (h == 0) { sts128<ST_B>(PA[0], uh[0], uh[1], uh[2], uh[3]); sts128<ST_B>(PA[1], 0u, 0u, 0u, 0u); }
            else { sts128<ST_B + 2 * (int)QBLK>(PA[0], ul[0], ul[1], ul[2], ul[3]); sts128<ST_B + 2 * (int)QBLK>(PA[1], 0u, 0u, 0u, 0u); }
        };
        auto load_w1 = [&]() {
            umma::fence_proxy_async();
            asm volatile("mbarrier.arrive.expect_tx.shared::cta.b64 _, [%0], %1;" ::"r"(umma::smem_u32(c.bars + B_W1)), "r"(2 * IMG_BLOCK) : "memory");
            asm volatile("cp.async.bulk.shared::cluster.global.mbarrier::complete_tx::bytes [%0], [%1], %2, [%3];"
                         ::"r"(umma::smem_u32(c.base + S_ST)), "l"(f.tc_img + IMG_W1_HI), "r"(2 * IMG_BLOCK), "r"(umma::smem_u32(c.bars + B_W1))
                         : "memory");
        };
        uint32_t* scr_p = scratch + (size_t)blockIdx.x * SCR_CTA_WORDS + p;
        auto load_z = [&](int r_hi, int r_lo, uint32_t (&wh)[2][16], uint32_t (&wl)[2][16]) {
#pragma unroll
            for (int cc = 0; cc < 2; ++cc) {
                umma::tmem_ld16(c.lane_base + (uint32_t)(r_hi + 16 * (2 * h + cc)), wh[cc]);
                umma::tmem_ld16(c.lane_base + (uint32_t)(r_lo + 16 * (2 * h + cc)), wl[cc]);
            }
            umma::wait_ld();
        };

        int64_t i_next = 0;
        { const int64_t s0 = (int64_t)blockIdx.x * TC_TP + p; if (s0 < N) i_next = am(s0); }
        for (int64_t tile = blockIdx.x; tile < n_tiles; tile += gridDim.x, ++k) {
            const int64_t slot = tile * TC_TP + p;
            const bool valid = slot < N;
            const int64_t i = i_next;
            { const int64_t s1 = slot + (int64_t)gridDim.x * TC_TP; i_next = s1 < N ? am(s1) : 0; }
            const uint32_t lay0 = 3u * k, prod0 = 5u * k;
            if (ctid == 0) {
                if (k > 0) {
                    c.ok &= umma::mbar_wait_spin(c.bars + B_FREE0 + 0, (prod0 - 1u) & 1u);
                    c.ok &= umma::mbar_wait_spin(c.bars + B_FREE0 + 2, (prod0 - 1u) & 1u);
                }
                load_w1();
            }
            B2_MARK(0);
            float g[3], gs[7];
            {
                const float2* gr = reinterpret_cast<const float2*>(d_raw + i * MF_RAW_DIM);
                float2 t2[5];
#pragma unroll
                for (int j = 0; j < 5; ++j) t2[j] = valid ? __ldg(gr + j) : make_float2(0.f, 0.f);
                g[0] = t2[0].x; g[1] = t2[0].y; g[2] = t2[1].x;
                gs[0] = t2[1].y; gs[1] = t2[2].x; gs[2] = t2[2].y; gs[3] = t2[3].x; gs[4] = t2[3].y; gs[5] = t2[4].x; gs[6] = t2[4].y;
            }
            float x[3] = {0.f, 0.f, 0.f};
            if (!f.feat && valid) src.point(i, f, x);
            const uint32_t* fin = f.feat ? f.feat + (size_t)(i >> 7) * FEAT_TILE_WORDS + (i & (TC_TP - 1)) : nullptr;
            auto e_words = [&](int qq, uint32_t (&hi)[8], uint32_t (&lo)[8]) {
                if (fin) {
                    const uint32_t* fq = fin + (size_t)qq * FEAT_WORDS * TC_TP;
#pragma unroll
                    for (int t = 0; t < 8; ++t) { hi[t] = __ldg(fq + t * TC_TP); lo[t] = __ldg(fq + (8 + t) * TC_TP); }
                } else {
                    float e[16];
                    tb_e_slots(x, qq, e);
#pragma unroll
                    for (int t = 0; t < 8; ++t) umma::split2(e[2 * t], e[2 * t + 1], hi[t], lo[t]);
                }
            };
#pragma unroll
            for (int sg = 0; sg < 2; ++sg) {
                const int qq = 2 * h + sg;
                uint32_t hi[8], lo[8], gh[4], gl[4];
                e_words(qq, hi, lo);
                if (fin) {
                    const uint32_t* fq = fin + (size_t)qq * FEAT_WORDS * TC_TP;
#pragma unroll
                    for (int t = 0; t < 4; ++t) { gh[t] = __ldg(fq + (16 + t) * TC_TP); gl[t] = __ldg(fq + (20 + t) * TC_TP); }
                } else {
                    float gf[8];
                    const float2* grid2 = reinterpret_cast<const float2*>(f.grid);
#pragma unroll
                    for (int ll = 0; ll < 4; ++ll) {
                        float2 vv = make_float2(0.f, 0.f);
                        if (valid) vv = grid_level_fwd(x, grid2, level_info(f, qq * 4 + ll), nullptr);
                        gf[2 * ll] = vv.x; gf[2 * ll + 1] = vv.y;
                    }
#pragma unroll
                    for (int t = 0; t < 4; ++t) umma::split2(gf[2 * t], gf[2 * t + 1], gh[t], gl[t]);
                }
                umma::tmem_st8(c.lane_base + T_R1_HI + 8 * qq, hi);
                umma::tmem_st8(c.lane_base + T_R1_LO + 8 * qq, lo);
                umma::tmem_st4(c.lane_base + T_G_HI + 4 * qq, gh);
                umma::tmem_st4(c.lane_base + T_G_LO + 4 * qq, gl);
            }
            B2_MARK(1);
            float v[32];
            uint32_t mask1[2], mask3[2];
            round([&]() {
                c.ok &= umma::mbar_wait_spin(c.bars + B_W1, k & 1u);
                issue_fwd<4>(c, W1H, W1L, [](int ks, bool lo) { return (lo ? T_R1_LO : T_R1_HI) + 8 * ks; });
            });
#pragma unroll 1
            for (int cc = 0; cc < 2; ++cc) {
                const int f0 = 64 * h + 32 * cc;
                ld32f(c.lane_base + T_D + f0, v);
                const float4* b4 = reinterpret_cast<const float4*>(c.fw + F_B1 + f0);
                uint32_t m = 0;
#pragma unroll
                for (int k4 = 0; k4 < 8; ++k4) {
                    const float4 b = b4[k4];
                    v[4 * k4] = fmaxf(v[4 * k4] + b.x, 0.f); v[4 * k4 + 1] = fmaxf(v[4 * k4 + 1] + b.y, 0.f);
                    v[4 * k4 + 2] = fmaxf(v[4 * k4 + 2] + b.z, 0.f); v[4 * k4 + 3] = fmaxf(v[4 * k4 + 3] + b.w, 0.f);
                }
#pragma unroll
                for (int kk = 0; kk < 32; ++kk) m |= (v[kk] > 0.f ? 1u : 0u) << kk;
                mask1[cc] = m;
                uint32_t hi[16], lo[16];
                split32(v, hi, lo);
                st_op(c, T_R1_HI, T_R1_LO, f0, hi, lo);
                scr_store(scr_p, SCR_H1, 64, f0 / 2, hi, lo);
            }
            B2_MARK(2);
            round([&]() { issue_fwd<8>(c, W2H, W2L, [](int ks, bool lo) { return (lo ? T_R1_LO : T_R1_HI) + 8 * ks; }); });
#pragma unroll 1
            for (int cc = 0; cc < 2; ++cc) {
                const int f0 = 64 * h + 32 * cc;
                ld32f(c.lane_base + T_D + f0, v);
                const float4* b4 = reinterpret_cast<const float4*>(c.fw + F_B2 + f0);
#pragma unroll
                for (int k4 = 0; k4 < 8; ++k4) {
                    const float4 b = b4[k4];
                    v[4 * k4] += b.x; v[4 * k4 + 1] += b.y; v[4 * k4 + 2] += b.z; v[4 * k4 + 3] += b.w;
                }
                uint32_t hi[16], lo[16];
                split32(v, hi, lo);
                if (h == 0) st_op(c, T_R2_HI, T_R2_LO, f0, hi, lo);
                else scr_store(scr_p, SCR_RGB, 32, 16 * cc, hi, lo);
            }
            B2_MARK(3);
            round([&]() {
                issue_fwd<6>(c, W3H, W3L, [](int ks, bool lo) {
                    return ks < 4 ? (lo ? T_R2_LO : T_R2_HI) + 8 * ks : (lo ? T_G_LO : T_G_HI) + 8 * (ks - 4);
                });
            });
            {
                float s[N_CLASS] = {0.f, 0.f, 0.f, 0.f, 0.f};
#pragma unroll 1
                for (int cc = 0; cc < 2; ++cc) {
                    const int f0 = 64 * h + 32 * cc;
                    ld32f(c.lane_base + T_D + f0, v);
                    const float4* b4 = reinterpret_cast<const float4*>(c.fw + F_BS1 + f0);
                    uint32_t m = 0;
#pragma unroll
                    for (int k4 = 0; k4 < 8; ++k4) {
                        const float4 b = b4[k4];
                        v[4 * k4] = fmaxf(v[4 * k4] + b.x, 0.f); v[4 * k4 + 1] = fmaxf(v[4 * k4 + 1] + b.y, 0.f);
                        v[4 * k4 + 2] = fmaxf(v[4 * k4 + 2] + b.z, 0.f); v[4 * k4 + 3] = fmaxf(v[4 * k4 + 3] + b.w, 0.f);
                    }
#pragma unroll
                    for (int kk = 0; kk < 32; ++kk) m |= (v[kk] > 0.f ? 1u : 0u) << kk;
                    mask3[cc] = m;
#pragma unroll
                    for (int ch = 0; ch < N_CLASS; ++ch) {
                        const float4* w4 = reinterpret_cast<const float4*>(c.fw + F_WS2 + ch * 128 + f0);
#pragma unroll
                        for (int k4 = 0; k4 < 8; ++k4) {
                            const float4 w = w4[k4];
                            s[ch] = fmaf(w.x, v[4 * k4], s[ch]); s[ch] = fmaf(w.y, v[4 * k4 + 1], s[ch]);
                            s[ch] = fmaf(w.z, v[4 * k4 + 2], s[ch]); s[ch] = fmaf(w.w, v[4 * k4 + 3], s[ch]);
                        }
                    }
                    uint32_t hi[16], lo[16];
                    split32(v, hi, lo);
                    scr_store(scr_p, SCR_H3, 64, f0 / 2, hi, lo);
                }
#pragma unroll
                for (int ch = 0; ch < N_CLASS; ++ch) c.part[(h * 5 + ch) * TC_LD + p] = s[ch];
            }
            B2_MARK(4);
            chain_sync();
            float dz4[N_CLASS];
            {
                float zl[N_CLASS], pr[N_CLASS], dp[N_CLASS];
                float mx = -INFINITY, se = 0.f, dot = 0.f;
#pragma unroll
                for (int ch = 0; ch < N_CLASS; ++ch) {
                    zl[ch] = c.fw[F_BS2 + ch] + (c.part[ch * TC_LD + p] + c.part[(5 + ch) * TC_LD + p]);
                    mx = fmaxf(mx, zl[ch]);
                }
#pragma unroll
                for (int ch = 0; ch < N_CLASS; ++ch) { pr[ch] = expf(zl[ch] - mx); se += pr[ch]; }
#pragma unroll
                for (int ch = 0; ch < N_CLASS; ++ch) {
                    pr[ch] = pr[ch] / se;
                    const float qq = pr[ch] + 1e-5f;
                    dp[ch] = gs[2 + ch] + gs[0] * (0.5f * (float)ch) - gs[1] * (log2f(qq) + pr[ch] / (qq * 0.6931471805599453f));
                    dot = fmaf(pr[ch], dp[ch], dot);
                }
#pragma unroll
                for (int ch = 0; ch < N_CLASS; ++ch) dz4[ch] = pr[ch] * (dp[ch] - dot);
            }
            uint32_t uh[4], ul[4];
            umma::split2(dz4[0], dz4[1], uh[0], ul[0]); umma::split2(dz4[2], dz4[3], uh[1], ul[1]);
            umma::split2(dz4[4], g[0], uh[2], ul[2]); umma::split2(g[1], g[2], uh[3], ul[3]);
#pragma unroll 1
            for (int cc = 0; cc < 2; ++cc) {
                const int f0 = 64 * h + 32 * cc;
#pragma unroll
                for (int kk = 0; kk < 32; ++kk) v[kk] = 0.f;
#pragma unroll
                for (int ch = 0; ch < N_CLASS; ++ch) {
                    const float4* w4 = reinterpret_cast<const float4*>(c.fw + F_WS2 + ch * 128 + f0);
                    const float dzc = dz4[ch];
#pragma unroll
                    for (int k4 = 0; k4 < 8; ++k4) {
                        const float4 w = w4[k4];
                        v[4 * k4] = fmaf(w.x, dzc, v[4 * k4]); v[4 * k4 + 1] = fmaf(w.y, dzc, v[4 * k4 + 1]);
                        v[4 * k4 + 2] = fmaf(w.z, dzc, v[4 * k4 + 2]); v[4 * k4 + 3] = fmaf(w.w, dzc, v[4 * k4 + 3]);
                    }
                }
                const uint32_t m = mask3[cc];
#pragma unroll
                for (int kk = 0; kk < 32; ++kk) v[kk] = ((m >> kk) & 1u) ? v[kk] : 0.f;
                uint32_t zh[16], zl[16];
                split32(v, zh, zl);
                st_op(c, T_R1_HI, T_R1_LO, f0, zh, zl);
            }
            B2_MARK(5);
            umma::wait_st();
            umma::fence_before_sync();
            chain_sync();
            if (ctid == 0) {
                umma::fence_after_sync();
                issue_dgrad<D_SDF_IN>(c, T_R1_HI, T_R1_LO, W3H, W3L);
                umma::commit(c.bars + B_DG3);
            }
            {
                uint32_t zh[2][16], zl[2][16], xh[2][16], xl[2][16];
                load_z(T_R1_HI, T_R1_LO, zh, zl);
                if (h == 0) {
#pragma unroll
                    for (int cc = 0; cc < 2; ++cc) { umma::tmem_ld16(c.lane_base + T_R2_HI + 16 * cc, xh[cc]); umma::tmem_ld16(c.lane_base + T_R2_LO + 16 * cc, xl[cc]); }
                } else {
                    umma::tmem_ld16(c.lane_base + T_G_HI, xh[0]); umma::tmem_ld16(c.lane_base + T_G_LO, xl[0]);
#pragma unroll
                    for (int t = 0; t < 16; ++t) { xh[1][t] = 0u; xl[1][t] = 0u; }
                    xh[1][0] = 0x00003F80u;
                }
                umma::wait_ld();
                if (prof && blockIdx.x == 0 && k == 1 && lane == 0 && h == 0) prof[32 + 4 * quarter] = clock64();
                prod_begin(prod0);
                if (prof && blockIdx.x == 0 && k == 1 && lane == 0 && h == 0) prof[33 + 4 * quarter] = clock64();
                put64<ST_A>(PH, zh, zl);
                put64<ST_B>(PH, xh, xl);
                if (prof && blockIdx.x == 0 && k == 1 && lane == 0 && h == 0) prof[34 + 4 * quarter] = clock64();
                prod_end(0, prod0, lay0);
                if (prof && blockIdx.x == 0 && k == 1 && lane == 0 && h == 0) prof[35 + 4 * quarter] = clock64();
#pragma unroll
                for (int cc = 0; cc < 2; ++cc) scr_load(scr_p, SCR_H3, 64, 32 * h + 16 * cc, zh[cc], zl[cc]);
                prod_begin(prod0 + 1u);
                put64<ST_A>(PH, zh, zl);
                put_u(uh, ul);
                prod_end(1, prod0 + 1u, lay0);
            }
            B2_MARK(6);
            c.ok &= umma::mbar_wait_spin(c.bars + B_DG3, k & 1u);
            umma::fence_after_sync();
            B2_MARK(7);
#pragma unroll 1
            for (int cc = 0; cc < 2; ++cc) {
                const int f0 = 64 * h + 32 * cc;
                if (h == 0) {
                    ld32f(c.lane_base + T_D + f0, v);
                } else {
                    const float* wr = c.fw + F_WR_EMB + 32 * cc;
#pragma unroll
                    for (int kk = 0; kk < 32; ++kk) v[kk] = fmaf(wr[128 + kk], g[2], fmaf(wr[64 + kk], g[1], wr[kk] * g[0]));
                }
                uint32_t zh[16], zl[16];
                split32(v, zh, zl);
                st_op(c, T_R2_HI, T_R2_LO, f0, zh, zl);
            }
            umma::wait_st();
            umma::fence_before_sync();
            chain_sync();
            if (ctid == 0) {
                c.ok &= umma::mbar_wait_spin(c.bars + B_DCONS, k & 1u);
                umma::fence_after_sync();
                issue_dgrad<D_H>(c, T_R2_HI, T_R2_LO, W2H, W2L);
                umma::commit(c.bars + B_MMA);
            }
            B2_MARK(8);
            {
                uint32_t ah[2][16], al[2][16], zh[2][16], zl[2][16];
#pragma unroll
                for (int cc = 0; cc < 2; ++cc) scr_load(scr_p, SCR_H1, 64, 32 * h + 16 * cc, ah[cc], al[cc]);
                load_z(T_R2_HI, T_R2_LO, zh, zl);
                prod_begin(prod0 + 2u);
                put64<ST_A>(PH, zh, zl);
                put64<ST_B>(PH, ah, al);
                prod_end(2, prod0 + 2u, lay0 + 1u);
            }
            c.ok &= umma::mbar_wait_spin(c.bars + B_MMA, ph_mma);
            ph_mma ^= 1;
            umma::fence_after_sync();
            B2_MARK(9);
#pragma unroll 1
            for (int cc = 0; cc < 2; ++cc) {
                const int f0 = 64 * h + 32 * cc;
                ld32f(c.lane_base + T_D + f0, v);
                const uint32_t m = mask1[cc];
#pragma unroll
                for (int kk = 0; kk < 32; ++kk) v[kk] = ((m >> kk) & 1u) ? v[kk] : 0.f;
                uint32_t zh[16], zl[16];
                split32(v, zh, zl);
                st_op(c, T_R1_HI, T_R1_LO, f0, zh, zl);
            }
            umma::wait_st();
            {
                uint32_t zh[2][16], zl[2][16], eh[2][8], el[2][8], rh[16], rl[16];
                load_z(T_R1_HI, T_R1_LO, zh, zl);
                e_words(2 * h, eh[0], el[0]); e_words(2 * h + 1, eh[1], el[1]);
                if (h == 0) { eh[0][7] = (eh[0][7] & 0x0000ffffu) | 0x3F800000u; el[0][7] &= 0x0000ffffu; }
                scr_load(scr_p, SCR_RGB, 32, 16 * h, rh, rl);
                prod_begin(prod0 + 3u);
                put64<ST_A>(PH, zh, zl);
#pragma unroll
                for (int sg = 0; sg < 2; ++sg)
#pragma unroll
                    for (int c_ = 0; c_ < 2; ++c_) {
                        sts128<ST_B>(PQ[2 * sg + c_], eh[sg][4 * c_], eh[sg][4 * c_ + 1], eh[sg][4 * c_ + 2], eh[sg][4 * c_ + 3]);
                        sts128<ST_B + 2 * (int)QBLK>(PQ[2 * sg + c_], el[sg][4 * c_], el[sg][4 * c_ + 1], el[sg][4 * c_ + 2], el[sg][4 * c_ + 3]);
                    }
                prod_end(3, prod0 + 3u, lay0 + 2u);
                prod_begin(prod0 + 4u);
#pragma unroll
                for (int sg = 0; sg < 2; ++sg)
#pragma unroll
                    for (int c_ = 0; c_ < 2; ++c_) {
                        sts128<ST_A>(PQ[2 * sg + c_], eh[sg][4 * c_], eh[sg][4 * c_ + 1], eh[sg][4 * c_ + 2], eh[sg][4 * c_ + 3]);
                        sts128<ST_A + 2 * (int)QBLK>(PQ[2 * sg + c_], el[sg][4 * c_], el[sg][4 * c_ + 1], el[sg][4 * c_ + 2], el[sg][4 * c_ + 3]);
                    }
#pragma unroll
                for (int c_ = 0; c_ < 4; ++c_) {
                    sts128<ST_A + (int)QBLK>(PQ[c_], rh[4 * c_], rh[4 * c_ + 1], rh[4 * c_ + 2], rh[4 * c_ + 3]);
                    sts128<ST_A + 3 * (int)QBLK>(PQ[c_], rl[4 * c_], rl[4 * c_ + 1], rl[4 * c_ + 2], rl[4 * c_ + 3]);
                }
                put_u(uh, ul);
                prod_end(4, prod0 + 4u, lay0 + 2u);
            }
            B2_MARK(10);
            umma::fence_before_sync();
            chain_sync();
        }
    } else if (ctid >= CHAIN_NT) {
        asm volatile("setmaxnreg.dec.sync.aligned.u32 %0;" ::"n"(REGS_WGRAD));
        const int wt = ctid - CHAIN_NT;
        const int kin = wt >= 64 ? wt - 64 : (tc_e_slot_to_index(wt) >= 0 ? 64 + tc_e_slot_to_index(wt) : -1);
        uint32_t k = 0, lay = 0;
        for (int64_t tile = blockIdx.x; tile < n_tiles; tile += gridDim.x, ++k) {
#pragma unroll 1
            for (int L = 0; L < 3; ++L, ++lay) {
                c.ok &= umma::mbar_wait_spin(c.bars + B_DWRDY, lay & 1u);
                umma::fence_after_sync();
                if (prof && blockIdx.x == 0 && k == 1 && wt == 0) prof[16 + L] = clock64();
                const int n_cols = L == 0 ? 128 : (L == 1 ? D_H : 80);
#pragma unroll 1
                for (int c0 = 0; c0 < n_cols; c0 += 16) {
                    uint32_t r[16];
                    umma::tmem_ld16(c.lane_base + (uint32_t)(T_DW + c0), r);
                    umma::wait_ld();
                    if (L == 1 || (L == 0 && c0 < D_SDF_IN)) {
                        float* dst = gpart + (L == 1 ? OFF_W2 : OFF_WS1) + c0 * D_H + wt;
#pragma unroll
                        for (int j = 0; j < 16; ++j) atomicAdd(dst + j * D_H, __uint_as_float(r[j]));
                    } else if (L == 0) {
                        if (c0 == D_SDF_IN) {
                            atomicAdd(&gpart[OFF_BS1 + wt], __uint_as_float(r[0]));
                        } else {
#pragma unroll
                            for (int j = 0; j < N_CLASS; ++j) atomicAdd(&gpart[OFF_WS2 + j * D_H + wt], __uint_as_float(r[j]));
                        }
                    } else if (c0 < 64) {
#pragma unroll
                        for (int j = 0; j < 16; ++j) {
                            const int ei = tc_e_slot_to_index(c0 + j);
                            if (ei >= 0) atomicAdd(&gpart[OFF_W1 + ei * D_H + wt], __uint_as_float(r[j]));
                            else if (c0 + j == 15) atomicAdd(&gpart[OFF_B1 + wt], __uint_as_float(r[j]));
                        }
                    } else if (wt == 15) {
#pragma unroll
                        for (int j = 0; j < N_CLASS; ++j) atomicAdd(&gpart[OFF_BS2 + j], __uint_as_float(r[j]));
#pragma unroll
                        for (int j = 0; j < 3; ++j) atomicAdd(&gpart[OFF_BR + j], __uint_as_float(r[N_CLASS + j]));
                    } else if (kin >= 0) {
#pragma unroll
                        for (int j = 0; j < 3; ++j) atomicAdd(&gpart[OFF_WR + j * D_RGB_IN + kin], __uint_as_float(r[N_CLASS + j]));
                    }
                }
                if (prof && blockIdx.x == 0 && k == 1 && wt == 0) prof[20 + L] = clock64();
                umma::fence_before_sync();
                umma::mbar_arrive(c.bars + B_DWFREE);
            }
        }
    } else {
        asm volatile("setmaxnreg.dec.sync.aligned.u32 %0;" ::"n"(REGS_SCATTER));
        uint32_t k = 0;
        for (int64_t tile = blockIdx.x; tile < n_tiles; tile += gridDim.x, ++k) {
            const int64_t slot = tile * TC_TP + p;
            const bool valid = slot < N;
            const int64_t i = valid ? am(slot) : 0;
            float x[3] = {0.f, 0.f, 0.f};
            if (valid) src.point(i, f, x);
            c.ok &= umma::mbar_wait_spin(c.bars + B_DG3, k & 1u);
            umma::fence_after_sync();
            if (prof && blockIdx.x == 0 && k == 1 && p == 0) prof[24] = clock64();
            uint32_t r[32];
            umma::tmem_ld32(c.lane_base + T_D + 64, r);
            umma::wait_ld();
            umma::fence_before_sync();
            umma::mbar_arrive(c.bars + B_DCONS);
            if (prof && blockIdx.x == 0 && k == 1 && p == 0) prof[26] = clock64();
#ifndef MF_EXP_NOSCATTER
            {
#pragma unroll 1
                for (int gq = 0; gq < 4; ++gq) {
                    float dy8[8];
#pragma unroll
                    for (int j = 0; j < 8; ++j)
                        dy8[j] = valid ? __uint_as_float(gq == 0 ? r[j] : (gq == 1 ? r[8 + j] : (gq == 2 ? r[16 + j] : r[24 + j]))) : 0.f;
#pragma unroll 1
                    for (int ll = 0; ll < 4; ++ll) {
                        const float2 dy = ll == 0 ? make_float2(dy8[0], dy8[1]) : (ll == 1 ? make_float2(dy8[2], dy8[3]) : (ll == 2 ? make_float2(dy8[4], dy8[5]) : make_float2(dy8[6], dy8[7])));
                        if (agg) grid_level_scatter_agg(x, dy, grad_grid, level_info(f, gq * 4 + ll), tid & 31);
                        else if (valid) { float dx[3]; grid_level_bwd<false>(x, dy, nullptr, grad_grid, level_info(f, gq * 4 + ll), dx); }
                    }
                }
            }
#endif
            if (prof && blockIdx.x == 0 && k == 1 && p == 0) prof[25] = clock64();
        }
    }
#undef B2_MARK
    if (!c.ok && err) atomicExch(err, 1);
    umma::fence_before_sync();
    __syncthreads();
    if (prof && tid == 0 && blockIdx.x < 256) prof[577 + 2 * blockIdx.x] = mf_globaltimer();
    if (warp == 0) umma::tmem_dealloc<512>(c.tmem);
}
```

mipsfusion_b200/csrc/field_tc_bwd3.cuh:

```cuda
#pragma once
#include <type_traits>
#include "field_tc_bwd2.cuh"

namespace b3 {

constexpr int B3_NT = 640, CHAIN_NT = 256, COPY_NT = 256, SC_NT = 128;
constexpr uint32_t QBLK = b2::QBLK;
constexpr int S_ST = IMG_F32;
constexpr int ST_A = b2::ST_A, ST_B = b2::ST_B, ST_BYTES = b2::ST_BYTES;
constexpr int S_F32 = S_ST + 2 * ST_BYTES;
constexpr int G_BS2 = F_WR_EMB + 192, G_COUNT = G_BS2 + 8;
static_assert(F_B1 == 0 && F_B2 == 128 && F_BS1 == 256 && F_WR_EMB == 384, "the first 576 floats of the image's fp32 section are copied as one block");
constexpr int S_BAR = S_F32 + G_COUNT * 4;
constexpr int S_BYTES = S_BAR + 256;
constexpr size_t SMEM = S_BYTES;
static_assert(SMEM <= 227 * 1024, "shared memory budget");
constexpr int SCR_U = b2::SCR_U;
constexpr int REGS_CHAIN = 112, REGS_COPY = 80;
using b2::T_D; using b2::T_R1_HI; using b2::T_R1_LO; using b2::T_R2_HI; using b2::T_R2_LO; using b2::T_DW; using b2::T_G_HI; using b2::T_G_LO;
using b2::SCR_H1; using b2::SCR_H3; using b2::SCR_RGB; using b2::SCR_CTA_WORDS; using b2::N_X3;
enum { B_MMA = 0, B_DG3, B_DCONS, B_DWRDY, B_Z3, B_ZH, B_Z1, B_RD0, B_RD2, B_RD3, B_RD4, B_FREE0, B_ISS0 = B_FREE0 + 4, B_COUNT = B_ISS0 + 4 };
static_assert(8 * B_COUNT + 8 <= 256, "barrier block");

__device__ __forceinline__ void chain_sync() { asm volatile("bar.sync 1, %0;" ::"n"(CHAIN_NT) : "memory"); }
__device__ __forceinline__ void copy_sync() { asm volatile("bar.sync 2, %0;" ::"n"(COPY_NT) : "memory"); }
template <int TILE_OFF, int CC>
__device__ __forceinline__ void put32h(const uint32_t (&PA)[8], uint32_t hq, const uint32_t (&pk)[16]) {
#pragma unroll
    for (int c_ = 0; c_ < 4; ++c_) b2::sts128<TILE_OFF>(PA[4 * CC + c_] + hq, pk[4 * c_], pk[4 * c_ + 1], pk[4 * c_ + 2], pk[4 * c_ + 3]);
}
__device__ __forceinline__ void warp_arrive(uint64_t* bar, int lane) {
    umma::fence_before_sync();
    __syncwarp();
    if (lane == 0) umma::mbar_arrive(bar);
}

}

template <class Src>
__global__ void __launch_bounds__(b3::B3_NT, 1) field_bwd_tc3_kernel(FieldDev f, Src src, const float* __restrict__ d_raw,
                                                                  float* __restrict__ grad_grid, float* __restrict__ part,
                                                                  uint32_t* __restrict__ scratch, int64_t N_all, ActiveMap am,
                                                                  int* __restrict__ err, long long* __restrict__ prof) {
    using namespace b3;
    extern __shared__ __align__(1024) uint8_t smem_raw[];
    const int tid = threadIdx.x, warp = tid >> 5, lane = tid & 31;
    float* gpart = part + (size_t)blockIdx.x * MF_MLP_PARAMS;
    for (int i = tid; i < MF_MLP_PARAMS; i += B3_NT) gpart[i] = 0.f;

    b2::Ctx c;
    c.base = smem_raw;
    c.ok = (umma::smem_u32(smem_raw) & 1023u) == 0u;
    c.fw = (const float*)(c.base + S_F32); c.part = nullptr; c.bars = (uint64_t*)(c.base + S_BAR);
    uint32_t* tmem_ptr = (uint32_t*)(c.base + S_BAR + 8 * B_COUNT);
    for (int i = tid; i < IMG_F32 / 16; i += B3_NT)
        reinterpret_cast<uint4*>(c.base)[i] = __ldg(reinterpret_cast<const uint4*>(f.tc_img) + i);
    for (int i = tid; i < (G_BS2 * 4) / 16 + 2; i += B3_NT) {
        const int src16 = i < (G_BS2 * 4) / 16 ? i : (F_BS2 * 4) / 16 + (i - (G_BS2 * 4) / 16);
        reinterpret_cast<uint4*>(c.base + S_F32)[i] = __ldg(reinterpret_cast<const uint4*>(f.tc_img + IMG_F32) + src16);
    }
    umma::fence_proxy_async();
    if (warp == 0) umma::tmem_alloc<512>(tmem_ptr);
    if (tid == 0) {
        umma::mbar_init(c.bars + B_MMA, 1); umma::mbar_init(c.bars + B_DG3, 1); umma::mbar_init(c.bars + B_DCONS, SC_NT);
        umma::mbar_init(c.bars + B_DWRDY, 4);
        umma::mbar_init(c.bars + B_Z3, 1); umma::mbar_init(c.bars + B_ZH, 1); umma::mbar_init(c.bars + B_Z1, CHAIN_NT / 32);
        umma::mbar_init(c.bars + B_RD0, COPY_NT / 32); umma::mbar_init(c.bars + B_RD2, COPY_NT / 32);
        umma::mbar_init(c.bars + B_RD3, COPY_NT / 32); umma::mbar_init(c.bars + B_RD4, COPY_NT / 32);
        for (int q = 0; q < 4; ++q) { umma::mbar_init(c.bars + B_FREE0 + q, 1); umma::mbar_init(c.bars + B_ISS0 + q, 1); }
        umma::fence_barrier_init();
    }
    umma::fence_before_sync();
    __syncthreads();
    umma::fence_after_sync();
    c.tmem = *tmem_ptr;
    c.lane_base = c.tmem + ((uint32_t)((warp & 3) * 32) << 16);

    const int64_t N = am.n(N_all);
    const int64_t n_tiles = (N + TC_TP - 1) / TC_TP;
    const int p = tid & (TC_TP - 1);
    uint32_t* scr_p = scratch + (size_t)blockIdx.x * SCR_CTA_WORDS + p;
#define B3_MARK(slot) do { if (prof && blockIdx.x == 0 && k == 1 && p == 0 && h == 0) prof[slot] = clock64(); } while (0)

    if (tid >= SC_NT + COPY_NT) {
        asm volatile("setmaxnreg.inc.sync.aligned.u32 %0;" ::"n"(REGS_CHAIN));
        const int ctid = tid - (SC_NT + COPY_NT), h = ctid >> 7;
        uint32_t ph_mma = 0;
        uint32_t k = 0;
        auto round = [&](auto issue) {
            umma::wait_st();
            umma::fence_before_sync();
            chain_sync();
            if (ctid == 0) { umma::fence_after_sync(); issue(); umma::commit(c.bars + B_MMA); }
            c.ok &= umma::mbar_wait_spin(c.bars + B_MMA, ph_mma);
            ph_mma ^= 1;
            umma::fence_after_sync();
        };
        const float4* ws2g = reinterpret_cast<const float4*>(f.tc_img + IMG_F32) + F_WS2 / 4;
        static_assert(F_WS2 % 4 == 0, "16-byte loads of sdf_linear.2.weight");

        int64_t i_next = 0;
        { const int64_t s0 = (int64_t)blockIdx.x * TC_TP + p; if (s0 < N) i_next = am(s0); }
        for (int64_t tile = blockIdx.x; tile < n_tiles; tile += gridDim.x, ++k) {
            const int64_t slot = tile * TC_TP + p;
            const bool valid = slot < N;
            const int64_t i = i_next;
            { const int64_t s1 = slot + (int64_t)gridDim.x * TC_TP; i_next = s1 < N ? am(s1) : 0; }
            const uint32_t pk = (k - 1u) & 1u;
            B3_MARK(0);
            float g[3], gs[7];
            {
                const float2* gr = reinterpret_cast<const float2*>(d_raw + i * MF_RAW_DIM);
                float2 t2[5];
#pragma unroll
                for (int j = 0; j < 5; ++j) t2[j] = valid ? __ldg(gr + j) : make_float2(0.f, 0.f);
                g[0] = t2[0].x; g[1] = t2[0].y; g[2] = t2[1].x;
                gs[0] = t2[1].y; gs[1] = t2[2].x; gs[2] = t2[2].y; gs[3] = t2[3].x; gs[4] = t2[3].y; gs[5] = t2[4].x; gs[6] = t2[4].y;
            }
            const uint32_t* fin = f.feat + (size_t)(i >> 7) * FEAT_TILE_WORDS + (i & (TC_TP - 1));
#pragma unroll
            for (int sg = 0; sg < 2; ++sg) {
                const int qq = 2 * h + sg;
                uint32_t hi[8], lo[8], gh[4], gl[4];
                const uint32_t* fq = fin + (size_t)qq * FEAT_WORDS * TC_TP;
#pragma unroll
                for (int t = 0; t < 8; ++t) { hi[t] = __ldg(fq + t * TC_TP); lo[t] = __ldg(fq + (8 + t) * TC_TP); }
#pragma unroll
                for (int t = 0; t < 4; ++t) { gh[t] = __ldg(fq + (16 + t) * TC_TP); gl[t] = __ldg(fq + (20 + t) * TC_TP); }
                if (sg == 0 && k > 0) {
                    c.ok &= umma::mbar_wait_spin(c.bars + B_RD3, pk);
                    c.ok &= umma::mbar_wait_spin(c.bars + B_RD2, pk);
                    umma::fence_after_sync();
                }
                umma::tmem_st8(c.lane_base + T_R1_HI + 8 * qq, hi);
                umma::tmem_st8(c.lane_base + T_R1_LO + 8 * qq, lo);
                umma::tmem_st4(c.lane_base + T_G_HI + 4 * qq, gh);
                umma::tmem_st4(c.lane_base + T_G_LO + 4 * qq, gl);
            }
            B3_MARK(1);
            float v[32];
            uint32_t mask1a = 0, mask1b = 0, mask3a = 0, mask3b = 0;
            round([&]() { b2::issue_fwd<4>(c, IMG_W1_HI, IMG_W1_LO, [](int ks, bool lo) { return (lo ? T_R1_LO : T_R1_HI) + 8 * ks; }); });
#pragma unroll 1
            for (int cc = 0; cc < 2; ++cc) {
                const int f0 = 64 * h + 32 * cc;
                b2::ld32f(c.lane_base + T_D + f0, v);
                const float4* b4 = reinterpret_cast<const float4*>(c.fw + F_B1 + f0);
                uint32_t m = 0;
#pragma unroll
                for (int k4 = 0; k4 < 8; ++k4) {
                    const float4 b = b4[k4];
                    v[4 * k4] = fmaxf(v[4 * k4] + b.x, 0.f); v[4 * k4 + 1] = fmaxf(v[4 * k4 + 1] + b.y, 0.f);
                    v[4 * k4 + 2] = fmaxf(v[4 * k4 + 2] + b.z, 0.f); v[4 * k4 + 3] = fmaxf(v[4 * k4 + 3] + b.w, 0.f);
                }
#pragma unroll
                for (int kk = 0; kk < 32; ++kk) m |= (v[kk] > 0.f ? 1u : 0u) << kk;
                if (cc == 0) mask1a = m; else mask1b = m;
                uint32_t hi[16], lo[16];
                b2::split32(v, hi, lo);
                b2::st_op(c, T_R1_HI, T_R1_LO, f0, hi, lo);
                b2::scr_store(scr_p, SCR_H1, 64, f0 / 2, hi, lo);
            }
            B3_MARK(2);
            round([&]() { b2::issue_fwd<8>(c, IMG_W2_HI, IMG_W2_LO, [](int ks, bool lo) { return (lo ? T_R1_LO : T_R1_HI) + 8 * ks; }); });
            if (k > 0) c.ok &= umma::mbar_wait_spin(c.bars + B_RD4, pk);
#pragma unroll 1
            for (int cc = 0; cc < 2; ++cc) {
                const int f0 = 64 * h + 32 * cc;
                b2::ld32f(c.lane_base + T_D + f0, v);
                const float4* b4 = reinterpret_cast<const float4*>(c.fw + F_B2 + f0);
#pragma unroll
                for (int k4 = 0; k4 < 8; ++k4) {
                    const float4 b = b4[k4];
                    v[4 * k4] += b.x; v[4 * k4 + 1] += b.y; v[4 * k4 + 2] += b.z; v[4 * k4 + 3] += b.w;
                }
                uint32_t hi[16], lo[16];
                b2::split32(v, hi, lo);
                if (h == 0) b2::st_op(c, T_R2_HI, T_R2_LO, f0, hi, lo);
                else b2::scr_store(scr_p, SCR_RGB, 32, 16 * cc, hi, lo);
            }
            B3_MARK(3);
            round([&]() {
                b2::issue_fwd<6>(c, IMG_W3_HI, IMG_W3_LO, [](int ks, bool lo) {
                    return ks < 4 ? (lo ? T_R2_LO : T_R2_HI) + 8 * ks : (lo ? T_G_LO : T_G_HI) + 8 * (ks - 4);
                });
            });
            float s[N_CLASS] = {0.f, 0.f, 0.f, 0.f, 0.f};
#pragma unroll 1
            for (int cc = 0; cc < 2; ++cc) {
                const int f0 = 64 * h + 32 * cc;
                b2::ld32f(c.lane_base + T_D + f0, v);
                const float4* b4 = reinterpret_cast<const float4*>(c.fw + F_BS1 + f0);
                uint32_t m = 0;
#pragma unroll
                for (int k4 = 0; k4 < 8; ++k4) {
                    const float4 b = b4[k4];
                    v[4 * k4] = fmaxf(v[4 * k4] + b.x, 0.f); v[4 * k4 + 1] = fmaxf(v[4 * k4 + 1] + b.y, 0.f);
                    v[4 * k4 + 2] = fmaxf(v[4 * k4 + 2] + b.z, 0.f); v[4 * k4 + 3] = fmaxf(v[4 * k4 + 3] + b.w, 0.f);
                }
#pragma unroll
                for (int kk = 0; kk < 32; ++kk) m |= (v[kk] > 0.f ? 1u : 0u) << kk;
                if (cc == 0) mask3a = m; else mask3b = m;
#pragma unroll
                for (int ch = 0; ch < N_CLASS; ++ch) {
                    const float4* w4 = ws2g + (ch * 128 + f0) / 4;
#pragma unroll
                    for (int k4 = 0; k4 < 8; ++k4) {
                        const float4 w = __ldg(w4 + k4);
                        s[ch] = fmaf(w.x, v[4 * k4], s[ch]); s[ch] = fmaf(w.y, v[4 * k4 + 1], s[ch]);
                        s[ch] = fmaf(w.z, v[4 * k4 + 2], s[ch]); s[ch] = fmaf(w.w, v[4 * k4 + 3], s[ch]);
                    }
                }
                uint32_t hi[16], lo[16];
                b2::split32(v, hi, lo);
                b2::scr_store(scr_p, SCR_H3, 64, f0 / 2, hi, lo);
            }
            float so[N_CLASS];
            {
                uint32_t sx[8] = {__float_as_uint(s[0]), __float_as_uint(s[1]), __float_as_uint(s[2]), __float_as_uint(s[3]), __float_as_uint(s[4]), 0u, 0u, 0u};
                umma::tmem_st8(c.lane_base + T_D + 64 * h, sx);
                umma::wait_st();
                umma::fence_before_sync();
                chain_sync();
                umma::fence_after_sync();
                uint32_t ox[8];
                umma::tmem_ld8(c.lane_base + T_D + 64 * (1 - h), ox);
                umma::wait_ld();
#pragma unroll
                for (int ch = 0; ch < N_CLASS; ++ch) so[ch] = __uint_as_float(ox[ch]);
            }
            B3_MARK(4);
            float dz4[N_CLASS];
            {
                float zl[N_CLASS], pr[N_CLASS], dp[N_CLASS];
                float mx = -INFINITY, se = 0.f, dot = 0.f;
#pragma unroll
                for (int ch = 0; ch < N_CLASS; ++ch) {
                    zl[ch] = c.fw[G_BS2 + ch] + (s[ch] + so[ch]);
                    mx = fmaxf(mx, zl[ch]);
                }
#pragma unroll
                for (int ch = 0; ch < N_CLASS; ++ch) { pr[ch] = expf(zl[ch] - mx); se += pr[ch]; }
#pragma unroll
                for (int ch = 0; ch < N_CLASS; ++ch) {
                    pr[ch] = pr[ch] / se;
                    const float qq = pr[ch] + 1e-5f;
                    dp[ch] = gs[2 + ch] + gs[0] * (0.5f * (float)ch) - gs[1] * (log2f(qq) + pr[ch] / (qq * 0.6931471805599453f));
                    dot = fmaf(pr[ch], dp[ch], dot);
                }
#pragma unroll
                for (int ch = 0; ch < N_CLASS; ++ch) dz4[ch] = pr[ch] * (dp[ch] - dot);
            }
            {
                uint32_t uh[4], ul[4];
                umma::split2(dz4[0], dz4[1], uh[0], ul[0]); umma::split2(dz4[2], dz4[3], uh[1], ul[1]);
                umma::split2(dz4[4], g[0], uh[2], ul[2]); umma::split2(g[1], g[2], uh[3], ul[3]);
#pragma unroll
                for (int t = 0; t < 4; ++t) __stcg(scr_p + (size_t)(SCR_U + 4 * h + t) * TC_TP, h ? ul[t] : uh[t]);
            }
#pragma unroll 1
            for (int cc = 0; cc < 2; ++cc) {
                const int f0 = 64 * h + 32 * cc;
#pragma unroll
                for (int kk = 0; kk < 32; ++kk) v[kk] = 0.f;
#pragma unroll
                for (int ch = 0; ch < N_CLASS; ++ch) {
                    const float4* w4 = ws2g + (ch * 128 + f0) / 4;
                    const float dzc = dz4[ch];
#pragma unroll
                    for (int k4 = 0; k4 < 8; ++k4) {
                        const float4 w = __ldg(w4 + k4);
                        v[4 * k4] = fmaf(w.x, dzc, v[4 * k4]); v[4 * k4 + 1] = fmaf(w.y, dzc, v[4 * k4 + 1]);
                        v[4 * k4 + 2] = fmaf(w.z, dzc, v[4 * k4 + 2]); v[4 * k4 + 3] = fmaf(w.w, dzc, v[4 * k4 + 3]);
                    }
                }
                const uint32_t m = cc == 0 ? mask3a : mask3b;
#pragma unroll
                for (int kk = 0; kk < 32; ++kk) v[kk] = ((m >> kk) & 1u) ? v[kk] : 0.f;
                uint32_t zh[16], zl[16];
                b2::split32(v, zh, zl);
                b2::st_op(c, T_R1_HI, T_R1_LO, f0, zh, zl);
            }
            B3_MARK(5);
            umma::wait_st();
            umma::fence_before_sync();
            __threadfence_block();
            chain_sync();
            if (ctid == 0) {
                umma::fence_after_sync();
                umma::mbar_arrive(c.bars + B_Z3);
                b2::issue_dgrad<D_SDF_IN>(c, T_R1_HI, T_R1_LO, IMG_W3_HI, IMG_W3_LO);
                umma::commit(c.bars + B_DG3);
            }
            c.ok &= umma::mbar_wait_spin(c.bars + B_DG3, k & 1u);
            c.ok &= umma::mbar_wait_spin(c.bars + B_RD0, k & 1u);
            umma::fence_after_sync();
            B3_MARK(6);
#pragma unroll 1
            for (int cc = 0; cc < 2; ++cc) {
                const int f0 = 64 * h + 32 * cc;
                if (h == 0) {
                    b2::ld32f(c.lane_base + T_D + f0, v);
                } else {
                    const float* wr = c.fw + F_WR_EMB + 32 * cc;
#pragma unroll
                    for (int kk = 0; kk < 32; ++kk) v[kk] = fmaf(wr[128 + kk], g[2], fmaf(wr[64 + kk], g[1], wr[kk] * g[0]));
                }
                uint32_t zh[16], zl[16];
                b2::split32(v, zh, zl);
                b2::st_op(c, T_R2_HI, T_R2_LO, f0, zh, zl);
            }
            umma::wait_st();
            umma::fence_before_sync();
            chain_sync();
            if (ctid == 0) {
                umma::fence_after_sync();
                umma::mbar_arrive(c.bars + B_ZH);
                c.ok &= umma::mbar_wait_spin(c.bars + B_DCONS, k & 1u);
                umma::fence_after_sync();
                b2::issue_dgrad<D_H>(c, T_R2_HI, T_R2_LO, IMG_W2_HI, IMG_W2_LO);
                umma::commit(c.bars + B_MMA);
            }
            B3_MARK(7);
            c.ok &= umma::mbar_wait_spin(c.bars + B_MMA, ph_mma);
            ph_mma ^= 1;
            umma::fence_after_sync();
            B3_MARK(8);
#pragma unroll 1
            for (int cc = 0; cc < 2; ++cc) {
                const int f0 = 64 * h + 32 * cc;
                b2::ld32f(c.lane_base + T_D + f0, v);
                const uint32_t m = cc == 0 ? mask1a : mask1b;
#pragma unroll
                for (int kk = 0; kk < 32; ++kk) v[kk] = ((m >> kk) & 1u) ? v[kk] : 0.f;
                uint32_t zh[16], zl[16];
                b2::split32(v, zh, zl);
                b2::st_op(c, T_R1_HI, T_R1_LO, f0, zh, zl);
            }
            umma::wait_st();
            warp_arrive(c.bars + B_Z1, lane);
            B3_MARK(9);
        }
    } else if (tid >= SC_NT) {
        asm volatile("setmaxnreg.dec.sync.aligned.u32 %0;" ::"n"(REGS_COPY));
        const int cp = tid - SC_NT, h = cp >> 7;
        const int row = p & (b2::QROWS - 1), quarter = p >> 5;
        const int kin = p >= 64 ? p - 64 : (tc_e_slot_to_index(p) >= 0 ? 64 + tc_e_slot_to_index(p) : -1);
        uint32_t PA[8];
#pragma unroll
        for (int j = 0; j < 8; ++j)
            PA[j] = umma::smem_u32(c.base) + (uint32_t)(S_ST + (quarter & 1) * ST_BYTES) + (uint32_t)((row >> 3) * 1024 + (row & 7) * 128) +
                    (uint32_t)(((j ^ row) & 7) << 4);
        const uint32_t hq = (uint32_t)h * QBLK;
        const uint64_t dA0 = umma::desc_mn(c.base + S_ST + (quarter & 1) * ST_BYTES + ST_A, 0, QBLK);
        const uint64_t dB0 = umma::desc_mn(c.base + S_ST + (quarter & 1) * ST_BYTES + ST_B, 0, QBLK);
        constexpr uint32_t LO_STEP = (2 * QBLK) >> 4, KS_STEP = (16 * 128) >> 4;
        auto prod_begin = [&](uint32_t prod) {
            c.ok &= umma::mbar_wait_spin(c.bars + B_FREE0 + ((quarter + 2) & 3), quarter >= 2 ? (prod & 1u) : ((prod + 1u) & 1u));
        };
        auto prod_end = [&](int PK, uint32_t prod) {
            umma::fence_proxy_async();
            asm volatile("bar.sync %0, 64;" ::"r"(3 + quarter) : "memory");
            if (h == 0 && lane == 0) {
                umma::fence_after_sync();
                if (quarter != 0) c.ok &= umma::mbar_wait_spin(c.bars + B_ISS0 + quarter - 1, prod & 1u);
                const int n_out = PK == 0 ? N_X3 : (PK == 2 ? D_H : (PK == 3 ? 64 : 16));
                const uint32_t idesc = umma::idesc_bf16(128, n_out, 1, 1);
                const uint32_t dcol = c.tmem + (uint32_t)(T_DW + (PK == 1 ? N_X3 : (PK == 4 ? 64 : 0)));
#pragma unroll
                for (int j = 0; j < 6; ++j) {
                    const int pass = j >> 1, ks = j & 1;
                    umma::mma_ss(dcol, dA0 + (uint64_t)((pass == 1 ? LO_STEP : 0) + ks * KS_STEP),
                                 dB0 + (uint64_t)((pass == 2 ? LO_STEP : 0) + ks * KS_STEP), idesc, (j == 0 && quarter == 0) ? 0u : 1u);
                }
                umma::mbar_arrive(c.bars + B_ISS0 + quarter);
                umma::commit(c.bars + B_FREE0 + quarter);
                if (PK == 1 || PK == 2 || PK == 4) umma::commit(c.bars + B_DWRDY);
            }
        };
        auto a_from_tmem = [&](int r_hi, int r_lo, uint32_t prod) {
#pragma unroll
            for (int cc = 0; cc < 2; ++cc) {
                uint32_t wh[16], wl[16];
                umma::tmem_ld16(c.lane_base + (uint32_t)(r_hi + 16 * (2 * h + cc)), wh);
                umma::tmem_ld16(c.lane_base + (uint32_t)(r_lo + 16 * (2 * h + cc)), wl);
                umma::wait_ld();
                if (cc == 0) prod_begin(prod);
                if (cc == 0) { put32h<ST_A, 0>(PA, hq, wh); put32h<ST_A + 2 * (int)QBLK, 0>(PA, hq, wl); }
                else { put32h<ST_A, 1>(PA, hq, wh); put32h<ST_A + 2 * (int)QBLK, 1>(PA, hq, wl); }
            }
        };
        auto from_scratch = [&](auto tile_off, int region, uint32_t prod, bool claim) {
            constexpr int TO = decltype(tile_off)::value;
#pragma unroll
            for (int cc = 0; cc < 2; ++cc) {
                uint32_t wh[16], wl[16];
                b2::scr_load(scr_p, region, 64, 32 * h + 16 * cc, wh, wl);
                if (cc == 0 && claim) prod_begin(prod);
                if (cc == 0) { put32h<TO, 0>(PA, hq, wh); put32h<TO + 2 * (int)QBLK, 0>(PA, hq, wl); }
                else { put32h<TO, 1>(PA, hq, wh); put32h<TO + 2 * (int)QBLK, 1>(PA, hq, wl); }
            }
        };
        auto put_u = [&]() {
            uint32_t u4[4];
#pragma unroll
            for (int t = 0; t < 4; ++t) u4[t] = __ldcg(scr_p + (size_t)(SCR_U + 4 * h + t) * TC_TP);
            if (h == 0) { b2::sts128<ST_B>(PA[0], u4[0], u4[1], u4[2], u4[3]); b2::sts128<ST_B>(PA[1], 0u, 0u, 0u, 0u); }
            else { b2::sts128<ST_B + 2 * (int)QBLK>(PA[0], u4[0], u4[1], u4[2], u4[3]); b2::sts128<ST_B + 2 * (int)QBLK>(PA[1], 0u, 0u, 0u, 0u); }
        };
        uint32_t lay = 0;
        auto read_out = [&](int L) {
            c.ok &= umma::mbar_wait_spin(c.bars + B_DWRDY, lay & 1u);
            umma::fence_after_sync();
            const int n_cols = L == 2 ? 80 : 128;
#pragma unroll 1
            for (int c0 = 16 * h; c0 < n_cols; c0 += 32) {
                uint32_t r[16];
                umma::tmem_ld16(c.lane_base + (uint32_t)(T_DW + c0), r);
                umma::wait_ld();
                if (L == 1 || (L == 0 && c0 < D_SDF_IN)) {
                    float* dst = gpart + (L == 1 ? OFF_W2 : OFF_WS1) + c0 * D_H + p;
#pragma unroll
                    for (int j = 0; j < 16; ++j) atomicAdd(dst + j * D_H, __uint_as_float(r[j]));
                } else if (L == 0) {
                    if (c0 == D_SDF_IN) {
                        atomicAdd(&gpart[OFF_BS1 + p], __uint_as_float(r[0]));
                    } else {
#pragma unroll
                        for (int j = 0; j < N_CLASS; ++j) atomicAdd(&gpart[OFF_WS2 + j * D_H + p], __uint_as_float(r[j]));
                    }
                } else if (c0 < 64) {
#pragma unroll
                    for (int j = 0; j < 16; ++j) {
                        const int ei = tc_e_slot_to_index(c0 + j);
                        if (ei >= 0) atomicAdd(&gpart[OFF_W1 + ei * D_H + p], __uint_as_float(r[j]));
                        else if (c0 + j == 15) atomicAdd(&gpart[OFF_B1 + p], __uint_as_float(r[j]));
                    }
                } else if (p == 15) {
#pragma unroll
                    for (int j = 0; j < N_CLASS; ++j) atomicAdd(&gpart[OFF_BS2 + j], __uint_as_float(r[j]));
#pragma unroll
                    for (int j = 0; j < 3; ++j) atomicAdd(&gpart[OFF_BR + j], __uint_as_float(r[N_CLASS + j]));
                } else if (kin >= 0) {
#pragma unroll
                    for (int j = 0; j < 3; ++j) atomicAdd(&gpart[OFF_WR + j * D_RGB_IN + kin], __uint_as_float(r[N_CLASS + j]));
                }
            }
            umma::fence_before_sync();
            copy_sync();
            ++lay;
        };
        using OffA = std::integral_constant<int, ST_A>;
        using OffB = std::integral_constant<int, ST_B>;

        uint32_t k = 0;
        for (int64_t tile = blockIdx.x; tile < n_tiles; tile += gridDim.x, ++k) {
            const int64_t slot = tile * TC_TP + p;
            const int64_t i = slot < N ? am(slot) : 0;
            const uint32_t* fin = f.feat + (size_t)(i >> 7) * FEAT_TILE_WORDS + (i & (TC_TP - 1));
            const uint32_t prod0 = 5u * k;
            c.ok &= umma::mbar_wait_spin(c.bars + B_Z3, k & 1u);
            umma::fence_after_sync();
            B3_MARK(16);
            a_from_tmem(T_R1_HI, T_R1_LO, prod0);
            if (h == 0) {
#pragma unroll
                for (int cc = 0; cc < 2; ++cc) {
                    uint32_t wh[16], wl[16];
                    umma::tmem_ld16(c.lane_base + T_R2_HI + 16 * cc, wh); umma::tmem_ld16(c.lane_base + T_R2_LO + 16 * cc, wl);
                    umma::wait_ld();
                    if (cc == 0) { put32h<ST_B, 0>(PA, hq, wh); put32h<ST_B + 2 * (int)QBLK, 0>(PA, hq, wl); }
                    else { put32h<ST_B, 1>(PA, hq, wh); put32h<ST_B + 2 * (int)QBLK, 1>(PA, hq, wl); }
                }
            } else {
                uint32_t wh[16], wl[16];
                umma::tmem_ld16(c.lane_base + T_G_HI, wh); umma::tmem_ld16(c.lane_base + T_G_LO, wl);
                umma::wait_ld();
                put32h<ST_B, 0>(PA, hq, wh); put32h<ST_B + 2 * (int)QBLK, 0>(PA, hq, wl);
#pragma unroll
                for (int t = 0; t < 16; ++t) { wh[t] = 0u; wl[t] = 0u; }
                wh[0] = 0x00003F80u;
                put32h<ST_B, 1>(PA, hq, wh); put32h<ST_B + 2 * (int)QBLK, 1>(PA, hq, wl);
            }
            warp_arrive(c.bars + B_RD0, lane);
            prod_end(0, prod0);
            B3_MARK(17);
            from_scratch(OffA{}, SCR_H3, prod0 + 1u, true);
            put_u();
            prod_end(1, prod0 + 1u);
            B3_MARK(18);
            read_out(0);
            B3_MARK(19);
            c.ok &= umma::mbar_wait_spin(c.bars + B_ZH, k & 1u);
            umma::fence_after_sync();
            B3_MARK(20);
            a_from_tmem(T_R2_HI, T_R2_LO, prod0 + 2u);
            warp_arrive(c.bars + B_RD2, lane);
            from_scratch(OffB{}, SCR_H1, 0u, false);
            prod_end(2, prod0 + 2u);
            B3_MARK(21);
            read_out(1);
            B3_MARK(22);
            c.ok &= umma::mbar_wait_spin(c.bars + B_Z1, k & 1u);
            umma::fence_after_sync();
            B3_MARK(23);
            a_from_tmem(T_R1_HI, T_R1_LO, prod0 + 3u);
            warp_arrive(c.bars + B_RD3, lane);
            auto put_e = [&](auto tile_off, int sg) {
                constexpr int TO = decltype(tile_off)::value;
                uint32_t eh[8], el[8];
                const uint32_t* fq = fin + (size_t)(2 * h + sg) * FEAT_WORDS * TC_TP;
#pragma unroll
                for (int t = 0; t < 8; ++t) { eh[t] = __ldg(fq + t * TC_TP); el[t] = __ldg(fq + (8 + t) * TC_TP); }
                if (h == 0 && sg == 0) { eh[7] = (eh[7] & 0x0000ffffu) | 0x3F800000u; el[7] &= 0x0000ffffu; }
#pragma unroll
                for (int c_ = 0; c_ < 2; ++c_) {
                    const uint32_t a = h ? PA[4 + 2 * sg + c_] : PA[2 * sg + c_];
                    b2::sts128<TO>(a, eh[4 * c_], eh[4 * c_ + 1], eh[4 * c_ + 2], eh[4 * c_ + 3]);
                    b2::sts128<TO + 2 * (int)QBLK>(a, el[4 * c_], el[4 * c_ + 1], el[4 * c_ + 2], el[4 * c_ + 3]);
                }
            };
            put_e(OffB{}, 0); put_e(OffB{}, 1);
            prod_end(3, prod0 + 3u);
            B3_MARK(24);
            {
                uint32_t rh[16], rl[16];
                b2::scr_load(scr_p, SCR_RGB, 32, 16 * h, rh, rl);
                prod_begin(prod0 + 4u);
#pragma unroll
                for (int c_ = 0; c_ < 4; ++c_) {
                    const uint32_t a = h ? PA[4 + c_] : PA[c_];
                    b2::sts128<ST_A + (int)QBLK>(a, rh[4 * c_], rh[4 * c_ + 1], rh[4 * c_ + 2], rh[4 * c_ + 3]);
                    b2::sts128<ST_A + 3 * (int)QBLK>(a, rl[4 * c_], rl[4 * c_ + 1], rl[4 * c_ + 2], rl[4 * c_ + 3]);
                }
            }
            put_e(OffA{}, 0); put_e(OffA{}, 1);
            put_u();
            warp_arrive(c.bars + B_RD4, lane);
            prod_end(4, prod0 + 4u);
            B3_MARK(25);
            read_out(2);
            B3_MARK(26);
        }
    } else {
        uint32_t k = 0;
        for (int64_t tile = blockIdx.x; tile < n_tiles; tile += gridDim.x, ++k) {
            const int64_t slot = tile * TC_TP + p;
            const bool valid = slot < N;
            const int64_t i = valid ? am(slot) : 0;
            float x[3] = {0.f, 0.f, 0.f};
            if (valid) src.point(i, f, x);
            c.ok &= umma::mbar_wait_spin(c.bars + B_DG3, k & 1u);
            umma::fence_after_sync();
            uint32_t r[32];
            umma::tmem_ld32(c.lane_base + T_D + 64, r);
            umma::wait_ld();
            umma::fence_before_sync();
            umma::mbar_arrive(c.bars + B_DCONS);
            if (prof && blockIdx.x == 0 && k == 1 && p == 0) prof[28] = clock64();
            if (valid) {
                float dx[3];
#pragma unroll 1
                for (int gq = 0; gq < 4; ++gq) {
                    float dy8[8];
#pragma unroll
                    for (int j = 0; j < 8; ++j)
                        dy8[j] = __uint_as_float(gq == 0 ? r[j] : (gq == 1 ? r[8 + j] : (gq == 2 ? r[16 + j] : r[24 + j])));
#pragma unroll
                    for (int ll = 0; ll < 4; ++ll)
                        grid_level_bwd<false>(x, make_float2(dy8[2 * ll], dy8[2 * ll + 1]), nullptr, grad_grid, level_info(f, gq * 4 + ll), dx);
                }
            }
            if (prof && blockIdx.x == 0 && k == 1 && p == 0) prof[29] = clock64();
        }
    }
#undef B3_MARK
    if (!c.ok && err) atomicExch(err, 1);
    umma::fence_before_sync();
    __syncthreads();
    if (warp == 0) umma::tmem_dealloc<512>(c.tmem);
}
```

mipsfusion_b200/csrc/mf_common.cuh:

```cuda
#pragma once
#include <cuda_runtime.h>
#include <stdint.h>
#include <stdio.h>
#include <string.h>

#include "../../include/mipsfusion_b200.h"

#define MF_API extern "C" __attribute__((visibility("default")))

void mf_set_error(const char* fmt, ...);

#define MF_CHECK_ARG(cond)                                                        \
    do {                                                                          \
        if (!(cond)) {                                                            \
            mf_set_error("%s: invalid argument: %s", __func__, #cond);            \
            return MF_ERR_INVALID;                                                \
        }                                                                         \
    } while (0)

#define MF_CUDA(expr)                                                             \
    do {                                                                          \
        cudaError_t _e = (expr);                                                  \
        if (_e != cudaSuccess) {                                                  \
            mf_set_error("%s: %s -> %s", __func__, #expr, cudaGetErrorString(_e)); \
            return MF_ERR_CUDA;                                                   \
        }                                                                         \
    } while (0)

#define MF_LAUNCH_CHECK() MF_CUDA(cudaGetLastError())

int mf_sm_count_cached();
constexpr int MF_KTIMER_SLOTS = 4;
void mf_ktimer_begin(int slot, cudaStream_t st);
void mf_ktimer_end(int slot, cudaStream_t st);

constexpr int TP = 64;
constexpr int LDA = TP + 4;
constexpr int NT = 256;

constexpr int D_GRID = 32;
constexpr int D_FREQ = 48;
constexpr int D_E = 51;
constexpr int D_EP = 52;
constexpr int D_H = 128;
constexpr int D_SDF_EMB = 64;
constexpr int D_RGB_IN = 115;
constexpr int D_SDF_IN = 96;
constexpr int N_CLASS = 5;

constexpr int OFF_W1 = 0;
constexpr int OFF_B1 = OFF_W1 + 128 * 51;
constexpr int OFF_W2 = OFF_B1 + 128;
constexpr int OFF_B2 = OFF_W2 + 128 * 128;
constexpr int OFF_WR = OFF_B2 + 128;
constexpr int OFF_BR = OFF_WR + 3 * 115;
constexpr int OFF_WS1 = OFF_BR + 3;
constexpr int OFF_BS1 = OFF_WS1 + 128 * 96;
constexpr int OFF_WS2 = OFF_BS1 + 128;
constexpr int OFF_BS2 = OFF_WS2 + 5 * 128;
static_assert(OFF_BS2 + 5 == MF_MLP_PARAMS, "decoder parameter count");

constexpr int PREP_RAW = 0;
constexpr int PREP_F1 = 36608;
constexpr int PREP_F2 = PREP_F1 + 52 * 128;
constexpr int PREP_F3 = PREP_F2 + 128 * 128;
constexpr int PREP_B1 = PREP_F3 + 96 * 128;
constexpr int PREP_B2 = PREP_B1 + 128 * 64;
constexpr int PREP_B3 = PREP_B2 + 128 * 128;
constexpr int PREP_SIMT_SIZE = PREP_B3 + 128 * 96;
constexpr int PREP_TC = PREP_SIMT_SIZE;
constexpr int PREP_SIZE = PREP_TC + 42388;
static_assert(PREP_F1 >= MF_MLP_PARAMS && PREP_F1 % 4 == 0 && PREP_TC % 4 == 0, "alignment");

struct FieldDev {
    const float* grid;
    const float* prep;
    const uint8_t* tc_img;
    uint32_t* feat;
    double na[3], nb[3], nf;
    int impl;
    int n_levels;
    float scale[MF_MAX_LEVELS];
    uint32_t res[MF_MAX_LEVELS], size[MF_MAX_LEVELS], offset[MF_MAX_LEVELS], hashed[MF_MAX_LEVELS];
};

struct ActiveMap {
    const int* idx; const int* count;
    __device__ __forceinline__ int64_t n(int64_t N) const { return count ? (int64_t)*count : N; }
    __device__ __forceinline__ int64_t operator()(int64_t slot) const { return idx ? (int64_t)idx[slot] : slot; }
};

int mf_field_to_dev(const mf_field* f, FieldDev* d);
int mf_decoder_impl();
int mf_bwd_impl();
int* mf_tc_error_flag();
int* mf_tile_counter();
int mf_sm_reserve();
constexpr int MF_PROF_SLOTS = 1024;
long long* mf_tc_profile_buffer();
__device__ __forceinline__ long long mf_globaltimer() { long long t; asm volatile("mov.u64 %0, %globaltimer;" : "=l"(t)); return t; }

__device__ __forceinline__ float warp_sum(float v) {
#pragma unroll
    for (int o = 16; o > 0; o >>= 1) v += __shfl_xor_sync(0xffffffffu, v, o);
    return v;
}
__device__ __forceinline__ double warp_sum_d(double v) {
#pragma unroll
    for (int o = 16; o > 0; o >>= 1) v += __shfl_xor_sync(0xffffffffu, v, o);
    return v;
}
__device__ __forceinline__ int warp_min_i(int v) {
#pragma unroll
    for (int o = 16; o > 0; o >>= 1) v = min(v, __shfl_xor_sync(0xffffffffu, v, o));
    return v;
}
__device__ __forceinline__ float sigmoidf_(float x) { return 1.0f / (1.0f + expf(-x)); }
```

Before: 7.229 million.

## Move decoder output heads (SDF logits and RGB) onto tcgen05 MMA

Adds a 16-wide bf16x3 head weight image (SDF class logits plus RGB weights) to the prepared tensor-core image. The forward and backward consumers now issue small N=16 UMMAs into a dedicated TMEM column range instead of computing per-thread FMA dot products and reducing partial sums through shared memory. This removes the SIMT head FMAs, the shared-memory partial buffers and a chain sync. In exchange it adds an extra MMA round, with its commit and wait, after layer 3, and it enlarges the weight image in shared memory and the prep buffer.

After: 7.390 million, median of 6. +2.2%, better.

```diff
diff --git a/mipsfusion_b200/csrc/field_kernels.cu b/mipsfusion_b200/csrc/field_kernels.cu
--- a/mipsfusion_b200/csrc/field_kernels.cu
+++ b/mipsfusion_b200/csrc/field_kernels.cu
@@ -53,8 +53,23 @@
         const uint32_t off = (uint32_t)(k >> 6) * IMG_BLOCK + sw128_offset(n, k & 63);
         *reinterpret_cast<__nv_bfloat16*>(img + hi_off + off) = h;
         *reinterpret_cast<__nv_bfloat16*>(img + lo_off + off) = l;
-    } else if (t < 128 * 320 + F_COUNT) {
-        const int j = t - 128 * 320;
+    } else if (t < 128 * 320 + HEAD_N * 256) {
+        const int r = t - 128 * 320, n = r / 256, k = r % 256;
+        float w = 0.f;
+        if (n < N_CLASS) {
+            if (k < D_H) w = mlp[OFF_WS2 + n * D_H + k];
+        } else if (n < N_CLASS + 3) {
+            const int c = n - N_CLASS;
+            if (k >= 128 && k < 192) w = mlp[OFF_WR + c * D_RGB_IN + (k - 128)];
+            else if (k >= 192) { const int e = tc_e_slot_to_index(k - 192); if (e >= 0) w = mlp[OFF_WR + c * D_RGB_IN + 64 + e]; }
+        }
+        const __nv_bfloat16 h = __float2bfloat16_rn(w);
+        const __nv_bfloat16 l = __float2bfloat16_rn(w - __bfloat162float(h));
+        const uint32_t off = (uint32_t)(k >> 6) * HEAD_BLOCK + sw128_offset(n, k & 63);
+        *reinterpret_cast<__nv_bfloat16*>(img + IMG_HEAD_HI + off) = h;
+        *reinterpret_cast<__nv_bfloat16*>(img + IMG_HEAD_LO + off) = l;
+    } else if (t < 128 * 320 + HEAD_N * 256 + F_COUNT) {
+        const int j = t - 128 * 320 - HEAD_N * 256;
         float v = 0.f;
         if (j < F_B2) v = mlp[OFF_B1 + j];
         else if (j < F_BS1) v = mlp[OFF_B2 + (j - F_B2)];
@@ -72,7 +87,8 @@
 }
 
 constexpr int PREP_BLOCKS_SIMT = (PREP_SIMT_SIZE + 255) / 256;
-constexpr int PREP_BLOCKS_TC = (128 * 320 + F_COUNT + 255) / 256;
+constexpr int PREP_BLOCKS_TC = (128 * 320 + HEAD_N * 256 + F_COUNT + 255) / 256;
+static_assert((PREP_SIZE - PREP_TC) * 4 >= IMG_BYTES, "mlp_prep holds the tensor-core weight image");
 __global__ void __launch_bounds__(256) mlp_prepare_kernel(const float* __restrict__ mlp, float* __restrict__ prep) {
     if (blockIdx.x < PREP_BLOCKS_SIMT) mlp_prepare_simt(mlp, prep, blockIdx.x * 256 + threadIdx.x);
     else mlp_prepare_tc(mlp, reinterpret_cast<uint8_t*>(prep + PREP_TC), (blockIdx.x - PREP_BLOCKS_SIMT) * 256 + threadIdx.x);
diff --git a/mipsfusion_b200/csrc/field_tc.cuh b/mipsfusion_b200/csrc/field_tc.cuh
--- a/mipsfusion_b200/csrc/field_tc.cuh
+++ b/mipsfusion_b200/csrc/field_tc.cuh
@@ -15,7 +15,11 @@
 constexpr int IMG_W2_LO = IMG_W2_HI + 2 * IMG_BLOCK;
 constexpr int IMG_W3_HI = IMG_W2_LO + 2 * IMG_BLOCK;
 constexpr int IMG_W3_LO = IMG_W3_HI + 2 * IMG_BLOCK;
-constexpr int IMG_F32 = IMG_W3_LO + 2 * IMG_BLOCK;
+constexpr int HEAD_N = 16, HEAD_BLOCK = HEAD_N * 128;
+constexpr int HEAD_KB_H3 = 0, HEAD_KB_EMB = 2, HEAD_KB_E = 3;
+constexpr int IMG_HEAD_HI = IMG_W3_LO + 2 * IMG_BLOCK;
+constexpr int IMG_HEAD_LO = IMG_HEAD_HI + 4 * HEAD_BLOCK;
+constexpr int IMG_F32 = IMG_HEAD_LO + 4 * HEAD_BLOCK;
 constexpr int F_B1 = 0, F_B2 = 128, F_BS1 = 256;
 constexpr int F_WR_EMB = 384;
 constexpr int F_WR_E = F_WR_EMB + 192;
diff --git a/mipsfusion_b200/csrc/field_tc3.cuh b/mipsfusion_b200/csrc/field_tc3.cuh
--- a/mipsfusion_b200/csrc/field_tc3.cuh
+++ b/mipsfusion_b200/csrc/field_tc3.cuh
@@ -4,11 +4,9 @@
 constexpr int T3_GT = 256;
 constexpr int T3_D = 0, T3_A_HI = 128, T3_A_LO = 192, T3_STG = 256, T3_STG_COLS = 96;
 constexpr int T3_E_HI = 0, T3_E_LO = 32, T3_G_HI = 64, T3_G_LO = 80;
-constexpr int T3_CPART_ROWS = 6;
-constexpr int T3_PART_ROWS = 13;
-constexpr int T3S_CPART = ((IMG_BYTES + 127) / 128) * 128;
-constexpr int T3S_PART = T3S_CPART + 2 * T3_CPART_ROWS * TC_LD * 4;
-constexpr int T3S_OUT = T3S_PART + T3_PART_ROWS * TC_LD * 4;
+constexpr int T3_HD = T3_STG + 2 * T3_STG_COLS;
+static_assert(T3_HD + HEAD_N <= 512, "tensor-memory budget");
+constexpr int T3S_OUT = ((IMG_BYTES + 127) / 128) * 128;
 constexpr int T3S_BAR = T3S_OUT + MF_RAW_DIM * TC_LD * 4;
 constexpr size_t SMEM_TC3 = T3S_BAR + 64 + 1024;
 static_assert(SMEM_TC3 <= 227 * 1024, "shared memory budget");
@@ -16,36 +14,57 @@
 __device__ __forceinline__ void t3_cons_sync() { asm volatile("bar.sync 1, %0;" ::"n"(T3_GT) : "memory"); }
 
 struct T3Cons {
-    uint8_t* img; const float* fw; float* part; float* out; uint64_t* bar;
+    uint8_t* img; const float* fw; float* out; uint64_t* bar;
     uint32_t tmem, lane_base, phase;
     int tid;
     bool ok;
 };
 
-template <int KS, int N_OUT = 128, class ColFn, class AfterFn>
-__device__ __forceinline__ void t3_run_layer(T3Cons& c, int img_hi, int img_lo, ColFn a_col, AfterFn after_issue) {
+template <class IssueFn, class AfterFn>
+__device__ __forceinline__ void t3_round(T3Cons& c, IssueFn issue, AfterFn after_commit) {
     umma::wait_st();
     umma::fence_before_sync();
     t3_cons_sync();
     if (c.tid == 0) {
         umma::fence_after_sync();
-        constexpr uint32_t idesc = umma::idesc_bf16(128, N_OUT, 0, 0);
-        const uint64_t dh = umma::smem_desc_sw128(umma::smem_u32(c.img + img_hi), 16, 1024);
-        const uint64_t dl = umma::smem_desc_sw128(umma::smem_u32(c.img + img_lo), 16, 1024);
-#pragma unroll
-        for (int pass = 0; pass < 3; ++pass) {
-#pragma unroll
-            for (int ks = 0; ks < KS; ++ks) {
-                const uint32_t off = (uint32_t)(((ks >> 2) * IMG_BLOCK + (ks & 3) * 32) >> 4);
-                umma::mma_ts(c.tmem + T3_D, c.tmem + (uint32_t)a_col(ks, pass == 2), (pass == 1 ? dl : dh) + off, idesc, (pass | ks) ? 1u : 0u);
-            }
-        }
+        issue();
         umma::commit(c.bar);
-        after_issue();
+        after_commit();
     }
     c.ok &= umma::mbar_wait(c.bar, c.phase);
     c.phase ^= 1;
     umma::fence_after_sync();
+}
+
+template <int KS, int N_OUT = 128, class ColFn>
+__device__ __forceinline__ void t3_issue_layer(const T3Cons& c, int img_hi, int img_lo, ColFn a_col) {
+    constexpr uint32_t idesc = umma::idesc_bf16(128, N_OUT, 0, 0);
+    const uint64_t dh = umma::smem_desc_sw128(umma::smem_u32(c.img + img_hi), 16, 1024);
+    const uint64_t dl = umma::smem_desc_sw128(umma::smem_u32(c.img + img_lo), 16, 1024);
+#pragma unroll
+    for (int pass = 0; pass < 3; ++pass) {
+#pragma unroll
+        for (int ks = 0; ks < KS; ++ks) {
+            const uint32_t off = (uint32_t)(((ks >> 2) * IMG_BLOCK + (ks & 3) * 32) >> 4);
+            umma::mma_ts(c.tmem + T3_D, c.tmem + (uint32_t)a_col(ks, pass == 2), (pass == 1 ? dl : dh) + off, idesc, (pass | ks) ? 1u : 0u);
+        }
+    }
+}
+
+template <int KS, bool ACC, class ColFn>
+__device__ __forceinline__ void t3_issue_head(const T3Cons& c, int kb, ColFn a_col) {
+    constexpr uint32_t idesc = umma::idesc_bf16(128, HEAD_N, 0, 0);
+    const uint64_t dh = umma::smem_desc_sw128(umma::smem_u32(c.img + IMG_HEAD_HI + kb * HEAD_BLOCK), 16, 1024);
+    const uint64_t dl = umma::smem_desc_sw128(umma::smem_u32(c.img + IMG_HEAD_LO + kb * HEAD_BLOCK), 16, 1024);
+#pragma unroll
+    for (int pass = 0; pass < 3; ++pass) {
+#pragma unroll
+        for (int ks = 0; ks < KS; ++ks) {
+            const uint32_t off = (uint32_t)(((ks >> 2) * HEAD_BLOCK + (ks & 3) * 32) >> 4);
+            umma::mma_ts(c.tmem + T3_HD, c.tmem + (uint32_t)a_col(ks, pass == 2), (pass == 1 ? dl : dh) + off, idesc,
+                         (ACC || pass || ks) ? 1u : 0u);
+        }
+    }
 }
 
 __device__ __forceinline__ void t3_load32(const T3Cons& c, int col, float (&v)[32]) {
@@ -110,7 +129,6 @@
         for (uint32_t k = 0;; ++k) {
             const int s = (int)(k & 1u);
             const uint32_t stg = lane_base + (uint32_t)(T3_STG + T3_STG_COLS * s);
-            float* cpart = (float*)(base + T3S_CPART) + s * T3_CPART_ROWS * TC_LD;
             T3_MARK(40);
             if (prof && blockIdx.x == 0 && tid == 0 && k < 12) prof[16 + k] = clock64();
             const int64_t tile_e = k < 2 ? (int64_t)blockIdx.x + (int64_t)k * gridDim.x : (int64_t)tq[k & 3u];
@@ -131,7 +149,6 @@
                 if (valid) src.point(i, f, x);
             }
             T3_MARK(41);
-            float r[3] = {0.f, 0.f, 0.f};
 #pragma unroll
             for (int sg = 0; sg < 2; ++sg) {
                 const int qq = 2 * h + sg;
@@ -152,17 +169,6 @@
 #pragma unroll
                     for (int t = 0; t < 8; ++t) { fo[t * TC_TP] = hi[t]; fo[(8 + t) * TC_TP] = lo[t]; }
                 }
-                if (!SDF_ONLY) {
-                    const float* wre = fw + F_WR_E + 16 * qq;
-#pragma unroll
-                    for (int t = 0; t < 16; ++t)
-#pragma unroll
-                        for (int ch = 0; ch < 3; ++ch) r[ch] = fmaf(wre[ch * 64 + t], e[t], r[ch]);
-                }
-            }
-            if (!SDF_ONLY) {
-#pragma unroll
-                for (int ch = 0; ch < 3; ++ch) cpart[(h * 3 + ch) * TC_LD + p] = r[ch];
             }
             T3_MARK(42);
 #pragma unroll 1
@@ -193,25 +199,22 @@
         }
     } else {
         T3Cons c;
-        c.img = base; c.fw = fw; c.part = (float*)(base + T3S_PART); c.out = (float*)(base + T3S_OUT); c.bar = bars;
+        c.img = base; c.fw = fw; c.out = (float*)(base + T3S_OUT); c.bar = bars;
         c.tmem = tmem; c.lane_base = lane_base; c.phase = 0; c.tid = tid; c.ok = ok;
         float v[32];
+        const auto a_region = [](int ks, bool lo) { return (lo ? T3_A_LO : T3_A_HI) + 8 * ks; };
         for (uint32_t k = 0;; ++k) {
             const int64_t tile = k < 2 ? (int64_t)blockIdx.x + (int64_t)k * gridDim.x : (int64_t)tq[k & 3u];
             if (tile >= n_tiles) break;
             const int s = (int)(k & 1u);
             const int stg = T3_STG + T3_STG_COLS * s;
-            const float* cpart = (const float*)(base + T3S_CPART) + s * T3_CPART_ROWS * TC_LD;
             T3_MARK(48);
             c.ok &= umma::mbar_wait(bars + 1 + s, (k >> 1) & 1u);
             umma::fence_after_sync();
             T3_MARK(49);
-            float rgb_e[3] = {0.f, 0.f, 0.f};
-            if (!SDF_ONLY && h == 0) {
-#pragma unroll
-                for (int ch = 0; ch < 3; ++ch) rgb_e[ch] = cpart[ch * TC_LD + p] + cpart[(3 + ch) * TC_LD + p];
-            }
-            t3_run_layer<4>(c, IMG_W1_HI, IMG_W1_LO, [stg](int ks, bool lo) { return stg + (lo ? T3_E_LO : T3_E_HI) + 8 * ks; }, []() {});
+            const auto a_e = [stg](int ks, bool lo) { return stg + (lo ? T3_E_LO : T3_E_HI) + 8 * ks; };
+            t3_round(c, [&]() { t3_issue_layer<4>(c, IMG_W1_HI, IMG_W1_LO, a_e); },
+                     [&]() { if (!SDF_ONLY) t3_issue_head<4, false>(c, HEAD_KB_E, a_e); });
             T3_MARK(50);
 #pragma unroll 1
             for (int half = 0; half < 2; ++half) {
@@ -228,7 +231,7 @@
             }
             T3_MARK(51);
             if (SDF_ONLY) {
-                t3_run_layer<8, 64>(c, IMG_W2_HI, IMG_W2_LO, [](int ks, bool lo) { return (lo ? T3_A_LO : T3_A_HI) + 8 * ks; }, []() {});
+                t3_round(c, [&]() { t3_issue_layer<8, 64>(c, IMG_W2_HI, IMG_W2_LO, a_region); }, []() {});
                 T3_MARK(52);
                 const int f0 = 32 * h;
                 t3_load32(c, T3_D + f0, v);
@@ -240,10 +243,8 @@
                 }
                 t3_store32(c, f0, v);
             } else {
-            t3_run_layer<8>(c, IMG_W2_HI, IMG_W2_LO, [](int ks, bool lo) { return (lo ? T3_A_LO : T3_A_HI) + 8 * ks; }, []() {});
-            T3_MARK(52);
-            {
-                float r[3] = {0.f, 0.f, 0.f};
+                t3_round(c, [&]() { t3_issue_layer<8>(c, IMG_W2_HI, IMG_W2_LO, a_region); }, []() {});
+                T3_MARK(52);
 #pragma unroll 1
                 for (int half = 0; half < 2; ++half) {
                     const int f0 = 64 * h + 32 * half;
@@ -254,90 +255,65 @@
                         const float4 b = b4[k4];
                         v[4 * k4] += b.x; v[4 * k4 + 1] += b.y; v[4 * k4 + 2] += b.z; v[4 * k4 + 3] += b.w;
                     }
-                    if (h == 0) {
-                        t3_store32(c, f0, v);
-                    } else {
-#pragma unroll
-                        for (int ch = 0; ch < 3; ++ch) {
-                            const float4* w4 = reinterpret_cast<const float4*>(c.fw + F_WR_EMB + ch * 64 + 32 * half);
-#pragma unroll
-                            for (int k4 = 0; k4 < 8; ++k4) {
-                                const float4 w = w4[k4];
-                                r[ch] = fmaf(w.x, v[4 * k4], r[ch]); r[ch] = fmaf(w.y, v[4 * k4 + 1], r[ch]);
-                                r[ch] = fmaf(w.z, v[4 * k4 + 2], r[ch]); r[ch] = fmaf(w.w, v[4 * k4 + 3], r[ch]);
-                            }
-                        }
-                    }
-                }
-                if (h == 1) {
-#pragma unroll
-                    for (int ch = 0; ch < 3; ++ch) c.part[ch * TC_LD + p] = r[ch];
-                }
-            }
+                    t3_store32(c, f0, v);
+                }
             }
             T3_MARK(53);
             uint64_t* empty = bars + 3 + s;
-            t3_run_layer<6>(c, IMG_W3_HI, IMG_W3_LO,
-                         [stg](int ks, bool lo) { return ks < 4 ? (lo ? T3_A_LO : T3_A_HI) + 8 * ks : stg + (lo ? T3_G_LO : T3_G_HI) + 8 * (ks - 4); },
-                         [empty]() { umma::commit(empty); });
+            t3_round(c, [&]() {
+                         t3_issue_layer<6>(c, IMG_W3_HI, IMG_W3_LO,
+                                           [stg](int ks, bool lo) { return ks < 4 ? (lo ? T3_A_LO : T3_A_HI) + 8 * ks : stg + (lo ? T3_G_LO : T3_G_HI) + 8 * (ks - 4); });
+                         if (!SDF_ONLY) t3_issue_head<4, true>(c, HEAD_KB_EMB, [](int ks, bool lo) { return (lo ? T3_A_LO : T3_A_HI) + 32 + 8 * ks; });
+                     },
+                     [empty]() { umma::commit(empty); });
             T3_MARK(54);
+#pragma unroll 1
+            for (int half = 0; half < 2; ++half) {
+                const int f0 = 64 * h + 32 * half;
+                t3_load32(c, T3_D + f0, v);
+                const float4* b4 = reinterpret_cast<const float4*>(c.fw + F_BS1 + f0);
+#pragma unroll
+                for (int k4 = 0; k4 < 8; ++k4) {
+                    const float4 b = b4[k4];
+                    v[4 * k4] = fmaxf(v[4 * k4] + b.x, 0.f); v[4 * k4 + 1] = fmaxf(v[4 * k4 + 1] + b.y, 0.f);
+                    v[4 * k4 + 2] = fmaxf(v[4 * k4 + 2] + b.z, 0.f); v[4 * k4 + 3] = fmaxf(v[4 * k4 + 3] + b.w, 0.f);
+                }
+                t3_store32(c, f0, v);
+            }
+            t3_round(c, [&]() { t3_issue_head<8, !SDF_ONLY>(c, HEAD_KB_H3, a_region); }, []() {});
+            T3_MARK(55);
             {
-                float sl[N_CLASS] = {0.f, 0.f, 0.f, 0.f, 0.f};
-#pragma unroll 1
-                for (int half = 0; half < 2; ++half) {
-                    const int f0 = 64 * h + 32 * half;
-                    t3_load32(c, T3_D + f0, v);
-                    const float4* b4 = reinterpret_cast<const float4*>(c.fw + F_BS1 + f0);
-#pragma unroll
-                    for (int k4 = 0; k4 < 8; ++k4) {
-                        const float4 b = b4[k4];
-                        v[4 * k4] = fmaxf(v[4 * k4] + b.x, 0.f); v[4 * k4 + 1] = fmaxf(v[4 * k4 + 1] + b.y, 0.f);
-                        v[4 * k4 + 2] = fmaxf(v[4 * k4 + 2] + b.z, 0.f); v[4 * k4 + 3] = fmaxf(v[4 * k4 + 3] + b.w, 0.f);
+                uint32_t r[8];
+                umma::tmem_ld8(c.lane_base + (uint32_t)T3_HD, r);
+                umma::wait_ld();
+                float* O = c.out;
+                if (h == 0) {
+                    float zl[N_CLASS];
+#pragma unroll
+                    for (int ch = 0; ch < N_CLASS; ++ch) zl[ch] = c.fw[F_BS2 + ch] + __uint_as_float(r[ch]);
+                    float mx = zl[0];
+#pragma unroll
+                    for (int ch = 1; ch < N_CLASS; ++ch) mx = fmaxf(mx, zl[ch]);
+                    float pr[N_CLASS], se = 0.f;
+#pragma unroll
+                    for (int ch = 0; ch < N_CLASS; ++ch) { pr[ch] = expf(zl[ch] - mx); se += pr[ch]; }
+                    float ent = 0.f, ex = 0.f;
+#pragma unroll
+                    for (int ch = 0; ch < N_CLASS; ++ch) {
+                        pr[ch] = pr[ch] / se;
+                        ent += pr[ch] * log2f(pr[ch] + 1e-5f);
+                        ex += pr[ch] * (float)ch;
                     }
-#pragma unroll
-                    for (int ch = 0; ch < N_CLASS; ++ch) {
-                        const float4* w4 = reinterpret_cast<const float4*>(c.fw + F_WS2 + ch * 128 + f0);
-#pragma unroll
-                        for (int k4 = 0; k4 < 8; ++k4) {
-                            const float4 w = w4[k4];
-                            sl[ch] = fmaf(w.x, v[4 * k4], sl[ch]); sl[ch] = fmaf(w.y, v[4 * k4 + 1], sl[ch]);
-                            sl[ch] = fmaf(w.z, v[4 * k4 + 2], sl[ch]); sl[ch] = fmaf(w.w, v[4 * k4 + 3], sl[ch]);
-                        }
-                    }
-                }
-#pragma unroll
-                for (int ch = 0; ch < N_CLASS; ++ch) c.part[(3 + h * 5 + ch) * TC_LD + p] = sl[ch];
-            }
-            T3_MARK(55);
+                    O[3 * TC_LD + p] = (ex / 4.0f - 0.5f) * 2.0f;
+                    O[4 * TC_LD + p] = -1.0f * ent;
+#pragma unroll
+                    for (int ch = 0; ch < N_CLASS; ++ch) O[(5 + ch) * TC_LD + p] = pr[ch];
+                } else {
+#pragma unroll
+                    for (int ch = 0; ch < 3; ++ch) O[ch * TC_LD + p] = SDF_ONLY ? 0.f : c.fw[F_BR + ch] + __uint_as_float(r[N_CLASS + ch]);
+                }
+            }
             umma::fence_before_sync();
-            t3_cons_sync();
-            if (h == 0) {
-                const float* P = c.part;
-                float zl[N_CLASS], rgb[3];
-#pragma unroll
-                for (int ch = 0; ch < N_CLASS; ++ch) zl[ch] = c.fw[F_BS2 + ch] + (P[(3 + ch) * TC_LD + p] + P[(8 + ch) * TC_LD + p]);
-#pragma unroll
-                for (int ch = 0; ch < 3; ++ch) rgb[ch] = SDF_ONLY ? 0.f : c.fw[F_BR + ch] + (rgb_e[ch] + P[ch * TC_LD + p]);
-                float mx = zl[0];
-#pragma unroll
-                for (int ch = 1; ch < N_CLASS; ++ch) mx = fmaxf(mx, zl[ch]);
-                float pr[N_CLASS], se = 0.f;
-#pragma unroll
-                for (int ch = 0; ch < N_CLASS; ++ch) { pr[ch] = expf(zl[ch] - mx); se += pr[ch]; }
-                float ent = 0.f, ex = 0.f;
-#pragma unroll
-                for (int ch = 0; ch < N_CLASS; ++ch) {
-                    pr[ch] = pr[ch] / se;
-                    ent += pr[ch] * log2f(pr[ch] + 1e-5f);
-                    ex += pr[ch] * (float)ch;
-                }
-                float* O = c.out;
-                O[0 * TC_LD + p] = rgb[0]; O[1 * TC_LD + p] = rgb[1]; O[2 * TC_LD + p] = rgb[2];
-                O[3 * TC_LD + p] = (ex / 4.0f - 0.5f) * 2.0f;
-                O[4 * TC_LD + p] = -1.0f * ent;
-#pragma unroll
-                for (int ch = 0; ch < N_CLASS; ++ch) O[(5 + ch) * TC_LD + p] = pr[ch];
-            }
             t3_cons_sync();
             T3_MARK(56);
             epi.store(c.out, TC_LD, TC_TP, tile, N, c.tid, T3_GT);
diff --git a/mipsfusion_b200/csrc/field_tc_bwd2.cuh b/mipsfusion_b200/csrc/field_tc_bwd2.cuh
--- a/mipsfusion_b200/csrc/field_tc_bwd2.cuh
+++ b/mipsfusion_b200/csrc/field_tc_bwd2.cuh
@@ -8,13 +8,12 @@
 constexpr uint32_t QBLK = QROWS * 128;
 constexpr int S_W = 0;
 constexpr int W2H = 0, W2L = IMG_W2_LO - IMG_W2_HI, W3H = IMG_W3_HI - IMG_W2_HI, W3L = IMG_W3_LO - IMG_W2_HI;
+constexpr int HDH = IMG_HEAD_HI - IMG_W2_HI, HDL = IMG_HEAD_LO - IMG_W2_HI;
 constexpr int S_ST = IMG_F32 - IMG_W2_HI;
 constexpr int ST_A = 0, ST_B = 4 * (int)QBLK, ST_BYTES = 8 * (int)QBLK;
 constexpr int W1H = S_ST + IMG_W1_HI, W1L = S_ST + IMG_W1_LO;
 constexpr int S_F32 = S_ST + 2 * ST_BYTES;
-constexpr int S_PART = S_F32 + ((F_COUNT * 4 + 127) / 128) * 128;
-constexpr int PART_ROWS = 10;
-constexpr int S_BAR = S_PART + PART_ROWS * TC_LD * 4;
+constexpr int S_BAR = S_F32 + ((F_COUNT * 4 + 127) / 128) * 128;
 constexpr int S_BYTES = S_BAR + 256;
 constexpr size_t SMEM = S_BYTES + 1024;
 static_assert(SMEM <= 227 * 1024, "shared memory budget");
@@ -30,7 +29,7 @@
 __device__ __forceinline__ void wg_sync() { asm volatile("bar.sync 2, %0;" ::"n"(WG_NT) : "memory"); }
 
 struct Ctx {
-    uint8_t* base; const float* fw; float* part; uint64_t* bars;
+    uint8_t* base; const float* fw; uint64_t* bars;
     uint32_t tmem, lane_base;
     bool ok;
 };
@@ -59,6 +58,19 @@
         for (int ks = 0; ks < 8; ++ks)
             umma::mma_ts(c.tmem + T_D, c.tmem + (uint32_t)((pass == 2 ? a_lo : a_hi) + 8 * ks), (pass == 1 ? dl : dh) + (uint32_t)((ks * 2048) >> 4),
                          idesc, (pass | ks) ? 1u : 0u);
+}
+
+__device__ __forceinline__ void issue_logits(const Ctx& c, int a_hi, int a_lo) {
+    constexpr uint32_t idesc = umma::idesc_bf16(128, HEAD_N, 0, 0);
+    const uint64_t dh = umma::smem_desc_sw128(umma::smem_u32(c.base + S_W + HDH), 16, 1024);
+    const uint64_t dl = umma::smem_desc_sw128(umma::smem_u32(c.base + S_W + HDL), 16, 1024);
+#pragma unroll
+    for (int pass = 0; pass < 3; ++pass)
+#pragma unroll
+        for (int ks = 0; ks < 8; ++ks) {
+            const uint32_t off = (uint32_t)(((ks >> 2) * HEAD_BLOCK + (ks & 3) * 32) >> 4);
+            umma::mma_ts(c.tmem + T_D, c.tmem + (uint32_t)((pass == 2 ? a_lo : a_hi) + 8 * ks), (pass == 1 ? dl : dh) + off, idesc, (pass | ks) ? 1u : 0u);
+        }
 }
 
 __device__ __forceinline__ void ld32f(uint32_t taddr, float (&v)[32]) {
@@ -129,7 +141,7 @@
 
     Ctx c;
     c.base = (uint8_t*)(((uintptr_t)smem_raw + 1023) & ~(uintptr_t)1023);
-    c.fw = (const float*)(c.base + S_F32); c.part = (float*)(c.base + S_PART); c.bars = (uint64_t*)(c.base + S_BAR);
+    c.fw = (const float*)(c.base + S_F32); c.bars = (uint64_t*)(c.base + S_BAR);
     uint32_t* tmem_ptr = (uint32_t*)(c.base + S_BAR + 8 * B_COUNT);
     if (warp == 0) umma::tmem_alloc<512>(tmem_ptr);
     if (tid == 0) {
@@ -351,49 +363,38 @@
                     return ks < 4 ? (lo ? T_R2_LO : T_R2_HI) + 8 * ks : (lo ? T_G_LO : T_G_HI) + 8 * (ks - 4);
                 });
             });
-            {
-                float s[N_CLASS] = {0.f, 0.f, 0.f, 0.f, 0.f};
-#pragma unroll 1
-                for (int cc = 0; cc < 2; ++cc) {
-                    const int f0 = 64 * h + 32 * cc;
-                    ld32f(c.lane_base + T_D + f0, v);
-                    const float4* b4 = reinterpret_cast<const float4*>(c.fw + F_BS1 + f0);
-                    uint32_t m = 0;
-#pragma unroll
-                    for (int k4 = 0; k4 < 8; ++k4) {
-                        const float4 b = b4[k4];
-                        v[4 * k4] = fmaxf(v[4 * k4] + b.x, 0.f); v[4 * k4 + 1] = fmaxf(v[4 * k4 + 1] + b.y, 0.f);
-                        v[4 * k4 + 2] = fmaxf(v[4 * k4 + 2] + b.z, 0.f); v[4 * k4 + 3] = fmaxf(v[4 * k4 + 3] + b.w, 0.f);
-                    }
-#pragma unroll
-                    for (int kk = 0; kk < 32; ++kk) m |= (v[kk] > 0.f ? 1u : 0u) << kk;
-                    mask3[cc] = m;
-#pragma unroll
-                    for (int ch = 0; ch < N_CLASS; ++ch) {
-                        const float4* w4 = reinterpret_cast<const float4*>(c.fw + F_WS2 + ch * 128 + f0);
-#pragma unroll
-                        for (int k4 = 0; k4 < 8; ++k4) {
-                            const float4 w = w4[k4];
-                            s[ch] = fmaf(w.x, v[4 * k4], s[ch]); s[ch] = fmaf(w.y, v[4 * k4 + 1], s[ch]);
-                            s[ch] = fmaf(w.z, v[4 * k4 + 2], s[ch]); s[ch] = fmaf(w.w, v[4 * k4 + 3], s[ch]);
-                        }
-                    }
-                    uint32_t hi[16], lo[16];
-                    split32(v, hi, lo);
-                    scr_store(scr_p, SCR_H3, 64, f0 / 2, hi, lo);
-                }
-#pragma unroll
-                for (int ch = 0; ch < N_CLASS; ++ch) c.part[(h * 5 + ch) * TC_LD + p] = s[ch];
-            }
+#pragma unroll 1
+            for (int cc = 0; cc < 2; ++cc) {
+                const int f0 = 64 * h + 32 * cc;
+                ld32f(c.lane_base + T_D + f0, v);
+                const float4* b4 = reinterpret_cast<const float4*>(c.fw + F_BS1 + f0);
+                uint32_t m = 0;
+#pragma unroll
+                for (int k4 = 0; k4 < 8; ++k4) {
+                    const float4 b = b4[k4];
+                    v[4 * k4] = fmaxf(v[4 * k4] + b.x, 0.f); v[4 * k4 + 1] = fmaxf(v[4 * k4 + 1] + b.y, 0.f);
+                    v[4 * k4 + 2] = fmaxf(v[4 * k4 + 2] + b.z, 0.f); v[4 * k4 + 3] = fmaxf(v[4 * k4 + 3] + b.w, 0.f);
+                }
+#pragma unroll
+                for (int kk = 0; kk < 32; ++kk) m |= (v[kk] > 0.f ? 1u : 0u) << kk;
+                mask3[cc] = m;
+                uint32_t hi[16], lo[16];
+                split32(v, hi, lo);
+                st_op(c, T_R1_HI, T_R1_LO, f0, hi, lo);
+                scr_store(scr_p, SCR_H3, 64, f0 / 2, hi, lo);
+            }
+            round([&]() { issue_logits(c, T_R1_HI, T_R1_LO); });
             B2_MARK(4);
-            chain_sync();
             float dz4[N_CLASS];
             {
                 float zl[N_CLASS], pr[N_CLASS], dp[N_CLASS];
                 float mx = -INFINITY, se = 0.f, dot = 0.f;
+                uint32_t r[8];
+                umma::tmem_ld8(c.lane_base + T_D, r);
+                umma::wait_ld();
 #pragma unroll
                 for (int ch = 0; ch < N_CLASS; ++ch) {
-                    zl[ch] = c.fw[F_BS2 + ch] + (c.part[ch * TC_LD + p] + c.part[(5 + ch) * TC_LD + p]);
+                    zl[ch] = c.fw[F_BS2 + ch] + __uint_as_float(r[ch]);
                     mx = fmaxf(mx, zl[ch]);
                 }
 #pragma unroll
diff --git a/mipsfusion_b200/csrc/field_tc_bwd3.cuh b/mipsfusion_b200/csrc/field_tc_bwd3.cuh
--- a/mipsfusion_b200/csrc/field_tc_bwd3.cuh
+++ b/mipsfusion_b200/csrc/field_tc_bwd3.cuh
@@ -6,7 +6,7 @@
 
 constexpr int B3_NT = 640, CHAIN_NT = 256, COPY_NT = 256, SC_NT = 128;
 constexpr uint32_t QBLK = b2::QBLK;
-constexpr int S_ST = IMG_F32;
+constexpr int S_ST = IMG_HEAD_HI;
 constexpr int ST_A = b2::ST_A, ST_B = b2::ST_B, ST_BYTES = b2::ST_BYTES;
 constexpr int S_F32 = S_ST + 2 * ST_BYTES;
 constexpr int G_BS2 = F_WR_EMB + 192, G_COUNT = G_BS2 + 8;
@@ -51,9 +51,9 @@
     b2::Ctx c;
     c.base = smem_raw;
     c.ok = (umma::smem_u32(smem_raw) & 1023u) == 0u;
-    c.fw = (const float*)(c.base + S_F32); c.part = nullptr; c.bars = (uint64_t*)(c.base + S_BAR);
+    c.fw = (const float*)(c.base + S_F32); c.bars = (uint64_t*)(c.base + S_BAR);
     uint32_t* tmem_ptr = (uint32_t*)(c.base + S_BAR + 8 * B_COUNT);
-    for (int i = tid; i < IMG_F32 / 16; i += B3_NT)
+    for (int i = tid; i < IMG_HEAD_HI / 16; i += B3_NT)
         reinterpret_cast<uint4*>(c.base)[i] = __ldg(reinterpret_cast<const uint4*>(f.tc_img) + i);
     for (int i = tid; i < (G_BS2 * 4) / 16 + 2; i += B3_NT) {
         const int src16 = i < (G_BS2 * 4) / 16 ? i : (F_BS2 * 4) / 16 + (i - (G_BS2 * 4) / 16);
diff --git a/mipsfusion_b200/csrc/mf_common.cuh b/mipsfusion_b200/csrc/mf_common.cuh
--- a/mipsfusion_b200/csrc/mf_common.cuh
+++ b/mipsfusion_b200/csrc/mf_common.cuh
@@ -69,7 +69,7 @@
 constexpr int PREP_B3 = PREP_B2 + 128 * 128;
 constexpr int PREP_SIMT_SIZE = PREP_B3 + 128 * 96;
 constexpr int PREP_TC = PREP_SIMT_SIZE;
-constexpr int PREP_SIZE = PREP_TC + 42388;
+constexpr int PREP_SIZE = PREP_TC + 46476;
 static_assert(PREP_F1 >= MF_MLP_PARAMS && PREP_F1 % 4 == 0 && PREP_TC % 4 == 0, "alignment");
 
 struct FieldDev {
```
